# abowman6/CBET_RayTracing_3D

Hardware: AMD Instinct MI355X
Metric: ray-steps/sec, OMEGA 60-beam 256^3 sweep (higher is better)
Workload: dtype f64

## Files before the change

cbet_raytracing_3d_amd/build.py:

```python
import os
import shutil
import subprocess
import sys

PKG = os.path.dirname(os.path.abspath(__file__))
ROOT = os.path.dirname(PKG)
CSRC = os.path.join(PKG, "csrc")
LIB_DIR = os.path.join(PKG, "lib")
LIB_PATH = os.path.join(LIB_DIR, "libcbet_mi355x.so")
SOURCES = ["cbet_kernels.hip", "cbet_trace_window.hip", "cbet_trace_exit.hip", "cbet_grid_kernels.hip", "cbet_sph_modes.hip",
           "cbet_target.hip", "cbet_mesh.hip", "cbet_mesh_deposit.hip", "cbet_params.cpp", "cbet_context.cpp", "cbet_tables_abi.cpp", "cbet_trace_abi.cpp", "cbet_gain_abi.cpp",
           "cbet_host.cpp", "cbet_output.cpp", "cbet_sph_host.cpp", "cbet_target_host.cpp", "cbet_mesh_host.cpp", "cbet_mesh_deposit_host.cpp",
           "cbet_exchange_host.cpp"]
HEADERS = [os.path.join(CSRC, "cbet_device.h"), os.path.join(CSRC, "cbet_host_internal.h"), os.path.join(CSRC, "cbet_relocate.h"), os.path.join(CSRC, "cbet_trace_common.h"), os.path.join(CSRC, "cbet_trace_diag.h"), os.path.join(CSRC, "cbet_hd.h"), os.path.join(CSRC, "cbet_node_model.h"), os.path.join(CSRC, "cbet_node_kernel.h"), os.path.join(CSRC, "cbet_target_model.h"), os.path.join(CSRC, "cbet_mesh_model.h"), os.path.join(CSRC, "cbet_state_model.h"), os.path.join(CSRC, "cbet_mesh_deposit_model.h"), os.path.join(CSRC, "cbet_gain_model.h"), os.path.join(ROOT, "include", "cbet_mi355x.h"),
           os.path.join(ROOT, "include", "cbet_omega_beams.h")]

FLAGS = ["-O3", "-std=c++17", "--offload-arch=gfx950", "-ffp-contract=off", "-fPIC", "-shared",
         "-Wall", "-Wextra", "-Wno-unused-result", "-mllvm", "-structurizecfg-skip-uniform-regions=true"]


def hipcc():
    exe = shutil.which("hipcc") or "/opt/rocm/bin/hipcc"
    if not os.path.exists(exe):
        raise RuntimeError("hipcc not found (need ROCm to build the gfx950 library)")
    return exe


def is_stale():
    if not os.path.exists(LIB_PATH):
        return True
    built = os.path.getmtime(LIB_PATH)
    deps = [os.path.join(CSRC, s) for s in SOURCES] + HEADERS + [os.path.abspath(__file__),
                                                                os.path.join(ROOT, "tools", "cbet_gpu.cpp"),
                                                                os.path.join(ROOT, "tools", "cbet_reference_shaped.cpp"),
                                                                os.path.join(ROOT, "include", "cbet_reference_api.hpp")]
    return any(os.path.getmtime(d) > built for d in deps)


def build(force=False, verbose=False, extra_flags=()):
    if not force and not is_stale():
        return LIB_PATH
    os.makedirs(LIB_DIR, exist_ok=True)
    cmd = [hipcc()] + FLAGS + list(extra_flags) + [
        "-I", os.path.join(ROOT, "include"), "-I", CSRC,
        "-o", LIB_PATH] + [os.path.join(CSRC, s) for s in SOURCES] + ["-lrccl"]
    if verbose:
        print(" ".join(cmd), flush=True)
    run = subprocess.run(cmd, stderr=subprocess.PIPE, text=True)
    sys.stderr.write(run.stderr)
    if run.returncode != 0 and "structurizecfg-skip-uniform-regions" in run.stderr:
        print("build: this hipcc does not know -structurizecfg-skip-uniform-regions; building without it", flush=True)
        k = cmd.index("-structurizecfg-skip-uniform-regions=true")
        subprocess.check_call(cmd[:k - 1] + cmd[k + 1:])
    elif run.returncode != 0:
        raise subprocess.CalledProcessError(run.returncode, cmd)
    build_cli(verbose)
    build_ref_shaped(verbose)
    return LIB_PATH


CLI_PATH = os.path.join(PKG, "lib", "cbet-gpu")


def build_cli(verbose=False):
    cmd = ["g++", "-O2", "-std=c++17", "-I", os.path.join(ROOT, "include"),
           os.path.join(ROOT, "tools", "cbet_gpu.cpp"), "-o", CLI_PATH,
           "-L", LIB_DIR, "-lcbet_mi355x", "-Wl,-rpath,$ORIGIN", "-Wl,-rpath-link," + "/opt/rocm/lib"]
    if verbose:
        print(" ".join(cmd), flush=True)
    subprocess.check_call(cmd)
    return CLI_PATH


REF_SHAPED_PATH = os.path.join(PKG, "lib", "cbet-ref-shaped")


def build_ref_shaped(verbose=False):
    cmd = [hipcc(), "-O2", "-std=c++17", "-I", os.path.join(ROOT, "include"),
           os.path.join(ROOT, "tools", "cbet_reference_shaped.cpp"), "-o", REF_SHAPED_PATH,
           "-L", LIB_DIR, "-lcbet_mi355x", "-Wl,-rpath,$ORIGIN"]
    if verbose:
        print(" ".join(cmd), flush=True)
    subprocess.check_call(cmd)
    return REF_SHAPED_PATH


def build_variant(name, extra_flags=(), verbose=False):
    out_dir = os.path.join(ROOT, "build_alt")
    os.makedirs(out_dir, exist_ok=True)
    out = os.path.join(out_dir, "libcbet_%s.so" % name)
    cmd = [hipcc()] + FLAGS + list(extra_flags) + ["-I", os.path.join(ROOT, "include"), "-I", CSRC, "-o", out] + \
        [os.path.join(CSRC, s) for s in SOURCES] + ["-lrccl"]
    if verbose:
        print(" ".join(cmd), flush=True)
    subprocess.check_call(cmd)
    return out


if __name__ == "__main__":
    if len(sys.argv) > 2 and sys.argv[1] == "--variant":
        print(build_variant(sys.argv[2], sys.argv[3:], verbose=True))
    else:
        print(build(force="--force" in sys.argv, verbose=True))
```

cbet_raytracing_3d_amd/csrc/cbet_context.cpp:

```cpp
#include <algorithm>
#include <cmath>
#include <cstring>
#include <map>
#include <mutex>
#include <vector>

#include "cbet_host_internal.h"

using namespace cbet;

int cbet::check_geometry(const cbet_context *ctx, const cbet_params *p)
{
    const cbet_params &q = ctx->p;
    if (p->nx != q.nx || p->ny != q.ny || p->nz != q.nz || p->xmin != q.xmin || p->xmax != q.xmax ||
        p->ymin != q.ymin || p->ymax != q.ymax || p->zmin != q.zmin || p->zmax != q.zmax ||
        p->rays_per_zone != q.rays_per_zone || p->nbeams != q.nbeams || p->nprofile != q.nprofile ||
        p->max_threads != q.max_threads || p->threads_per_block != q.threads_per_block ||
        p->courant_mult != q.courant_mult || p->patch_order != q.patch_order || p->rim_merge != q.rim_merge)
        return fail(CBET_EINVAL, "launch parameters do not match the geometry the context was created for");
    return CBET_OK;
}

int cbet::entry_checks(const cbet_context *ctx, const cbet_params *p)
{
    if (!ctx) return fail(CBET_EINVAL, "NULL context");
    if (int rc = validate(p)) return rc;
    return check_geometry(ctx, p);
}

static std::mutex g_ctx_mu;
static std::map<int, cbet_context *> g_default_ctx;

int cbet::default_context(const cbet_params *p, cbet_context **out)
{
    int dev = 0;
    CBET_HIP(hipGetDevice(&dev));
    std::lock_guard<std::mutex> lk(g_ctx_mu);
    auto it = g_default_ctx.find(dev);
    if (it != g_default_ctx.end()) {
        if (check_geometry(it->second, p) == CBET_OK) {
            *out = it->second;
            return CBET_OK;
        }
        cbet_context_destroy(it->second);
        g_default_ctx.erase(it);
    }
    cbet_context *ctx = nullptr;
    if (int rc = cbet_context_create(&ctx, p, dev)) return rc;
    g_default_ctx[dev] = ctx;
    *out = ctx;
    return CBET_OK;
}

extern "C" {

int cbet_safeGPUAlloc(void **dst, size_t size, int gpu)
{
    if (!dst) return fail(CBET_EINVAL, "dst is NULL");
    hipError_t e = hipSetDevice(gpu);
    if (e != hipSuccess) return fail_hip(CBET_ENODEVICE, "hipSetDevice(%d): %s", gpu, hipGetErrorString(e));
    size_t free_b = 0, total_b = 0;
    e = hipMemGetInfo(&free_b, &total_b);
    if (e != hipSuccess) return fail_hip(CBET_EHIP, "Error encountered during hipMemGetInfo: %s", hipGetErrorString(e));
    if (free_b < size) return fail_hip(CBET_ENOMEM, "GPU: %d is out of memory", gpu);
    e = hipMalloc(dst, size);
    if (e != hipSuccess) return fail_hip(CBET_EHIP, "Error encountered during hipMalloc: %s", hipGetErrorString(e));
    return CBET_OK;
}

int cbet_moveToAndFromGPU(void *dst, void *src, size_t size, int gpu)
{
    if (gpu == -1) return fail_hip(CBET_ENODEVICE, "Attempting to move data that has not been assigned a GPU");
    if (size && (!dst || !src)) return fail(CBET_EINVAL, "NULL pointer");
    DeviceGuard guard;
    hipError_t e = hipSetDevice(gpu);
    if (e != hipSuccess) return fail_hip(CBET_ENODEVICE, "hipSetDevice(%d): %s", gpu, hipGetErrorString(e));
    e = hipMemcpy(dst, src, size, hipMemcpyDefault);
    if (e != hipSuccess) return fail_hip(CBET_EHIP, "Error encountered during hipMemcpy: %s", hipGetErrorString(e));
    return CBET_OK;
}

int cbet_gpuFree(void *ptr, int gpu)
{
    DeviceGuard guard;
    hipError_t e = hipSetDevice(gpu);
    if (e != hipSuccess) return fail_hip(CBET_ENODEVICE, "hipSetDevice(%d): %s", gpu, hipGetErrorString(e));
    CBET_HIP(hipFree(ptr));
    return CBET_OK;
}

int cbet_context_destroy(cbet_context *ctx)
{
    if (!ctx) return CBET_OK;
    DeviceGuard guard;
    (void)hipSetDevice(ctx->gpu);
    (void)hipFree(ctx->ne3d);
    (void)hipFree(ctx->kap3d);
    (void)hipFree(ctx->steprec);
    (void)hipFree(ctx->xlaunch);
    (void)hipFree(ctx->ylaunch);
    (void)hipFree(ctx->bounds);
    (void)hipFree(ctx->live);
    (void)hipFree(ctx->counters);
    (void)hipFree(ctx->flow_own);
    (void)hipFree(ctx->state_own);
    (void)hipFree(ctx->shift_own);
    delete ctx;
    return CBET_OK;
}

int cbet_context_set_launch_list(cbet_context *ctx, const int *list, long n)
{
    if (!ctx || !list) return fail(CBET_EINVAL, "NULL context or list");
    if (n <= 0 || n % kWave != 0) return fail(CBET_EINVAL, "a launch list is a whole number of 64-entry bundles (got %ld entries)", n);
    CBET_ENTER_DEVICE(ctx);
    CBET_HIP(hipDeviceSynchronize());
    std::vector<int> cur((size_t)ctx->nlive), want, got;
    if (ctx->nlive) CBET_HIP(hipMemcpy(cur.data(), ctx->live, cur.size() * sizeof(int), hipMemcpyDeviceToHost));
    for (int v : cur) if (v >= 0) want.push_back(v);
    for (long i = 0; i < n; ++i) {
        if (list[i] >= 0) got.push_back(list[i]);
        else if (list[i] != -1) return fail(CBET_EINVAL, "launch list entry %ld is %d (a ray id or -1)", i, list[i]);
    }
    for (long b = 0; b < n; b += kWave) {
        bool any = false;
        for (int l = 0; l < kWave; ++l) any = any || list[b + l] >= 0;
        if (!any) return fail(CBET_EINVAL, "bundle %ld of the launch list is empty", b / kWave);
    }
    std::sort(want.begin(), want.end());
    std::sort(got.begin(), got.end());
    if (want != got) return fail(CBET_EINVAL, "the launch list must hold exactly the context's live rays, each once (%zu given, %zu expected)", got.size(), want.size());
    int *fresh = nullptr;
    CBET_HIP(hipMalloc((void **)&fresh, (size_t)n * sizeof(int)));
    hipError_t e = hipMemcpy(fresh, list, (size_t)n * sizeof(int), hipMemcpyHostToDevice);
    if (e != hipSuccess) { (void)hipFree(fresh); return fail_hip(CBET_EHIP, "hipMemcpy(launch list): %s", hipGetErrorString(e)); }
    (void)hipFree(ctx->live);
    ctx->live = fresh;
    ctx->nlive = (int)n;
    return CBET_OK;
}

int cbet_context_create(cbet_context **out, const cbet_params *p, int gpu)
{
    if (!out) return fail(CBET_EINVAL, "ctx out-pointer is NULL");
    *out = nullptr;
    cbet_derived d;
    std::vector<double> xl, yl;
    std::vector<int> live;
    if (int rc = derive_launch(p, &d, xl, yl, live)) return rc;

    DeviceGuard guard;
    hipError_t e = hipSetDevice(gpu);
    if (e != hipSuccess) return fail_hip(CBET_ENODEVICE, "hipSetDevice(%d): %s", gpu, hipGetErrorString(e));
    cbet_context *ctx = new cbet_context;
    ctx->gpu = gpu;
    ctx->p = *p;
    ctx->d = d;
    ctx->nlive = (int)live.size();
    const size_t nodes = (size_t)p->nx * p->ny * p->nz;
    auto bail = [&](hipError_t err, const char *what) {
        cbet_context_destroy(ctx);
        return fail_hip(err == hipErrorOutOfMemory ? CBET_ENOMEM : CBET_EHIP, "%s: %s", what, hipGetErrorString(err));
    };
    if ((e = hipMalloc((void **)&ctx->ne3d, nodes * sizeof(double))) != hipSuccess) return bail(e, "hipMalloc(ne3d)");
    if ((e = hipMalloc((void **)&ctx->kap3d, nodes * sizeof(double))) != hipSuccess) return bail(e, "hipMalloc(kappa3d)");
    if ((e = hipMalloc((void **)&ctx->steprec, nodes * sizeof(StepRecord))) != hipSuccess) return bail(e, "hipMalloc(step records)");
    if ((e = hipMalloc((void **)&ctx->xlaunch, xl.size() * sizeof(double))) != hipSuccess) return bail(e, "hipMalloc(xlaunch)");
    if ((e = hipMalloc((void **)&ctx->ylaunch, yl.size() * sizeof(double))) != hipSuccess) return bail(e, "hipMalloc(ylaunch)");
    if ((e = hipMalloc((void **)&ctx->bounds, 6 * sizeof(double))) != hipSuccess) return bail(e, "hipMalloc(bounds)");
    {
        double hb[6];
        host_exit_planes(p, d, hb);
        if ((e = hipMemcpy(ctx->bounds, hb, sizeof hb, hipMemcpyHostToDevice)) != hipSuccess) return bail(e, "hipMemcpy(bounds)");
    }
    if ((e = hipMalloc((void **)&ctx->live, std::max<size_t>(1, live.size()) * sizeof(int))) != hipSuccess) return bail(e, "hipMalloc(live)");
    if ((e = hipMalloc((void **)&ctx->counters, kCntSlots * sizeof(unsigned long long))) != hipSuccess) return bail(e, "hipMalloc(counters)");
    if ((e = hipMemcpy(ctx->xlaunch, xl.data(), xl.size() * sizeof(double), hipMemcpyHostToDevice)) != hipSuccess) return bail(e, "hipMemcpy(xlaunch)");
    if ((e = hipMemcpy(ctx->ylaunch, yl.data(), yl.size() * sizeof(double), hipMemcpyHostToDevice)) != hipSuccess) return bail(e, "hipMemcpy(ylaunch)");
    if (!live.empty() &&
        (e = hipMemcpy(ctx->live, live.data(), live.size() * sizeof(int), hipMemcpyHostToDevice)) != hipSuccess)
        return bail(e, "hipMemcpy(live)");
    if ((e = hipMemset(ctx->counters, 0, kCntSlots * sizeof(unsigned long long))) != hipSuccess) return bail(e, "hipMemset(counters)");
    if ((e = target_upload_factors()) != hipSuccess) return bail(e, "hipMemcpyToSymbol(target factors)");
    *out = ctx;
    return CBET_OK;
}

int cbet_context_counters(cbet_context *ctx, void *stream, cbet_counters *out, int reset)
{
    if (!ctx || !out) return fail(CBET_EINVAL, "NULL context/counters");
    CBET_ENTER_DEVICE(ctx);
    hipStream_t s = (hipStream_t)stream;
    unsigned long long h[kCntSlots];
    CBET_HIP(hipMemcpyAsync(h, ctx->counters, sizeof h, hipMemcpyDeviceToHost, s));
    if (reset) CBET_HIP(hipMemsetAsync(ctx->counters, 0, sizeof h, s));
    CBET_HIP(hipStreamSynchronize(s));
    std::memset(out, 0, sizeof *out);
    out->ray_steps = h[kCntSteps];
    out->rays_traced = h[kCntRays];
    out->global_atomics = h[kCntGlobalAtomics];
    out->lds_evictions = h[kCntEvictions];
    out->wave_steps = h[kCntWaveSteps];
    out->wave_steps_miss = h[kCntWaveStepsMiss];
    out->wave_steps_wide = h[kCntWaveStepsWide];
    out->slabs_retired = h[kCntSlabsRetired];
    return CBET_OK;
}

int cbet_debug_bounds_violations(unsigned long long *out, int reset, void *stream)
{
    if (!out) return fail(CBET_EINVAL, "out is NULL");
    hipError_t e = audit_violations(out, reset != 0, (hipStream_t)stream);
    if (e == hipErrorNotSupported) return fail(CBET_EINVAL, "not a bounds-audit build (compile with -DCBET_DEBUG_BOUNDS)");
    if (e != hipSuccess) return fail_hip(CBET_EHIP, "audit_violations: %s", hipGetErrorString(e));
    return CBET_OK;
}

int cbet_context_list_length(const cbet_context *ctx, long *length)
{
    if (!ctx || !length) return fail(CBET_EINVAL, "NULL context/length");
    *length = ctx->nlive;
    return CBET_OK;
}

int cbet_context_tables(cbet_context *ctx, double **ne3d, double **kappa3d)
{
    if (!ctx) return fail(CBET_EINVAL, "NULL context");
    if (ne3d) *ne3d = ctx->ne3d;
    if (kappa3d) *kappa3d = ctx->kap3d;
    ++ctx->tables_version;
    return CBET_OK;
}

int cbet_context_step_records(const cbet_context *ctx, const void **records, unsigned long long *builds)
{
    if (!ctx) return fail(CBET_EINVAL, "NULL context");
    if (records) *records = ctx->steprec;
    if (builds) *builds = ctx->rec_builds;
    return CBET_OK;
}

int cbet_context_set_flow(cbet_context *ctx, const double *flow)
{
    if (!ctx) return fail(CBET_EINVAL, "NULL context");
    ctx->flow = flow;
    return CBET_OK;
}

int cbet_context_flow(cbet_context *ctx, void **out)
{
    if (!ctx || !out) return fail(CBET_EINVAL, "NULL context/out");
    *out = const_cast<double *>(ctx->flow);
    return CBET_OK;
}

int cbet_context_set_state(cbet_context *ctx, const double *state)
{
    if (!ctx) return fail(CBET_EINVAL, "NULL context");
    ctx->state = state;
    return CBET_OK;
}

int cbet_context_state(cbet_context *ctx, void **out)
{
    if (!ctx || !out) return fail(CBET_EINVAL, "NULL context/out");
    *out = const_cast<double *>(ctx->state);
    return CBET_OK;
}

int cbet_context_set_saturation(cbet_context *ctx, double dn_max)
{
    if (std::isnan(dn_max)) return fail(CBET_EINVAL, "cbet_context_set_saturation: dn_max is NaN (a finite limit > 0, or 0 = none)");
    if (std::isinf(dn_max)) return fail(CBET_EINVAL, "cbet_context_set_saturation: dn_max is infinite (a finite limit > 0, or 0 = none)");
    if (dn_max < 0.0) return fail(CBET_EINVAL, "cbet_context_set_saturation: dn_max = %g is negative (a finite limit > 0, or 0 = none)", dn_max);
    if (!ctx) return fail(CBET_EINVAL, "NULL context");
    ctx->dn_max = dn_max;
    return CBET_OK;
}

int cbet_context_saturation(cbet_context *ctx, double *out)
{
    if (!ctx || !out) return fail(CBET_EINVAL, "NULL context/out");
    *out = ctx->dn_max;
    return CBET_OK;
}

int cbet_context_set_detuning(cbet_context *ctx, const double *domega, int nbeams, void *stream)
{
    if (domega) {
        if (nbeams > CBET_MAX_CBET_BEAMS)
            return fail(CBET_EINVAL, "cbet_context_set_detuning: nbeams = %d exceeds CBET_MAX_CBET_BEAMS = %d", nbeams, CBET_MAX_CBET_BEAMS);
        if (nbeams < 1) return fail(CBET_EINVAL, "cbet_context_set_detuning: nbeams = %d (one shift per beam)", nbeams);
        for (int b = 0; b < nbeams; ++b) {
            if (std::isnan(domega[b])) return fail(CBET_EINVAL, "cbet_context_set_detuning: domega[%d] is NaN (finite shifts in rad/s, or NULL = none)", b);
            if (std::isinf(domega[b])) return fail(CBET_EINVAL, "cbet_context_set_detuning: domega[%d] is infinite (finite shifts in rad/s, or NULL = none)", b);
        }
    }
    if (!ctx) return fail(CBET_EINVAL, "NULL context");
    if (domega && nbeams != ctx->p.nbeams)
        return fail(CBET_EINVAL, "cbet_context_set_detuning: nbeams = %d, the context was created for %d beams", nbeams, ctx->p.nbeams);
    bool one_colour = true;
    for (int b = 1; domega && b < nbeams; ++b) one_colour = one_colour && domega[b] == domega[0];
    if (one_colour) {
        ctx->shift = nullptr;
        return CBET_OK;
    }
    CBET_ENTER_DEVICE(ctx);
    if (!ctx->shift_own) {
        hipError_t e = hipMalloc((void **)&ctx->shift_own, sizeof ctx->shift_host);
        if (e != hipSuccess) {
            ctx->shift_own = nullptr;
            return fail_hip(e == hipErrorOutOfMemory ? CBET_ENOMEM : CBET_EHIP, "hipMalloc(detuning table): %s", hipGetErrorString(e));
        }
    }
    double fresh[CBET_MAX_CBET_BEAMS] = {};
    for (int b = 0; b < nbeams; ++b) fresh[b] = domega[b];
    CBET_HIP(hipStreamSynchronize((hipStream_t)stream));
    CBET_HIP(hipMemcpy(ctx->shift_own, fresh, sizeof fresh, hipMemcpyHostToDevice));
    std::memcpy(ctx->shift_host, fresh, sizeof fresh);
    ctx->shift = ctx->shift_own;
    return CBET_OK;
}

int cbet_context_detuning(cbet_context *ctx, double *out, int *nbeams)
{
    if (!ctx || !nbeams) return fail(CBET_EINVAL, "NULL context/nbeams");
    *nbeams = ctx->shift ? ctx->p.nbeams : 0;
    if (out)
        for (int b = 0; b < *nbeams; ++b) out[b] = ctx->shift_host[b];
    return CBET_OK;
}

}
```

cbet_raytracing_3d_amd/csrc/cbet_device.h:

```cpp
#ifndef CBET_DEVICE_H_
#define CBET_DEVICE_H_

#include <hip/hip_runtime_api.h>

#include "cbet_mi355x.h"

namespace cbet {

constexpr double kC = 29979245800.0;
constexpr double kE0 = 8.85418782e-12;
constexpr double kMe = 9.10938356e-31;
constexpr double kEc = 1.60217662e-19;
constexpr double kLambda = 1.053e-4 / 3.0;
constexpr double kSigma = 0.0375;
constexpr double kIntensity = 1.0e14;
constexpr double kFocal = 0.1;
constexpr double kBeamMin = -450.0e-4;
constexpr double kBeamMax = 450.0e-4;

constexpr unsigned kEmptyTag = 0xFFFFFFFFu;
constexpr int kWave = 64;

enum CounterSlot { kCntSteps = 0, kCntRays = 1, kCntGlobalAtomics = 2, kCntEvictions = 3, kCntWaveSteps = 4,
                   kCntWaveStepsMiss = 5, kCntWaveStepsWide = 6, kCntSlabsRetired = 7, kCntSlots = 8 };

struct TabulateArgs {
    int nx, ny, nz, nprofile;
    double xmin, ymin, zmin;
    double dx, dy, dz, dt;
    double ncrit;
    const double *r, *ne, *te;
    double *ne3d, *kap3d;
};

struct StepRecord {
    double kx, ky, kz, kap;
};

struct StepTableArgs {
    int nx, ny, nz;
    double xconst, yconst, zconst;
    const double *ne3d, *kap3d;
    StepRecord *rec;
};

struct PlasmaRecordsArgs {
    TabulateArgs t;
    double xconst, yconst, zconst;
    StepRecord *rec;
};

struct TraceArgs {
    int nx, ny, nz;
    double xmin, ymin, zmin;
    double dx, dy, dz, dt;
    double inv_dx, inv_dy, inv_dz;
    double fx_hi, fy_hi, fz_hi;
    const double *bounds;
    double exit_planes[6];
    double tol_x, tol_y, tol_z;
    double xconst, yconst, zconst;
    int nt, absorption;
    int rpz, zones, nrays_x;
    double z_launch;
    double uray_mult, omega, ncrit;
    const double *xlaunch, *ylaunch;
    const int *live;
    int nlive;
    int beam_lo, nbeams_local, bundles_per_beam;
    long total_bundles;
    long first_item, item_count;
    const double *ne3d, *kap3d;
    const StepRecord *steprec;
    const double *beam_norm, *bbeam_norm, *pow_r, *phase_r;
    double *edep;
    int sYh, sXh;
    long grid_stride;
    unsigned long long *counters;
    int stats;
    unsigned long long *audit_count;
    const double *audit_lo, *audit_hi;
    unsigned long long audit_nodes, audit_hsize;
    int grid_beam0;
    const double *gain;
    long hsize;
    int quantity;
    long comp_stride;
    double max_exponent;
    double *beam_gain;
};

struct GainArgs {
    int nx, ny, nz, nbeams;
    double xmin, ymin, zmin, dx, dy, dz, dt;
    double ncrit, k0;
    double cs, gain_const, iaw;
    double mach_r0, mach_0, mach_r1, mach_1;
    double relax;
    double *fields;
    const double *ne3d;
    double *gain;
    double *scratch;
    double *change;
    int hx_lo, hx_hi;
    int consume;
    int frozen;
    long store0, bstride;
    const double *flow;
    const double *state;
    double sat;
    const double *shift;
};

hipError_t launch_tabulate(const TabulateArgs &a, hipStream_t stream);
hipError_t launch_step_table(const StepTableArgs &a, hipStream_t stream);
hipError_t launch_plasma_records(const PlasmaRecordsArgs &a, hipStream_t stream);
size_t plasma_records_lds(int nprofile);
hipError_t audit_violations(unsigned long long *out, bool reset, hipStream_t stream);
hipError_t launch_trace(const TraceArgs &a, int variant, bool force_idx64, hipStream_t stream);
hipError_t launch_trace_window(const TraceArgs &a, bool force_idx64, hipStream_t stream);
constexpr int kTraceExits = 100;
constexpr int kExitDoubles = 10;
hipError_t launch_trace_exit(const TraceArgs &a, bool force_idx64, hipStream_t stream);
hipError_t launch_exit_tally(const cbet_ray_exit *exits, long L, int nbeams, double *tally, hipStream_t stream);
hipError_t launch_farfield(const cbet_ray_exit *exits, long n, int ntheta, int nphi, double *hist, hipStream_t stream);
hipError_t launch_gain_field(const GainArgs &a, hipStream_t stream);
hipError_t launch_pair_amplitude(const GainArgs &a, double *amp, hipStream_t stream);
inline long exchange_groups(long rows) { return rows < CBET_EXCHANGE_MAX_GROUPS ? rows : CBET_EXCHANGE_MAX_GROUPS; }
hipError_t launch_exchange_matrix(const GainArgs &a, double *work, double *out, double *gross, hipStream_t stream);
hipError_t launch_pack_segments(const double *src, long beam_stride, int hy, int hz, const int *seg, long nseg, double *out,
                                hipStream_t stream);
hipError_t launch_unpack_segments(double *dst, long beam_stride, int hy, int hz, const int *seg, long nseg, const double *in,
                                  hipStream_t stream);
hipError_t launch_edep_average(const double *edep, double *out, int nx, int ny, int nz, hipStream_t stream);

struct SphArgs {
    const double *edep;
    long grid_stride;
    long row_pitch;
    int ngrids, nx, ny, nz;
    int nshell, lmax;
    double xmin, ymin, zmin, dx, dy, dz;
    double cx, cy, cz;
    double *coeffs;
    double *shell_energy;
    long long *shell_nodes;
    double r_edges[CBET_SPH_MAX_SHELLS + 1];
};
hipError_t launch_sph_modes(const SphArgs &a, hipStream_t stream);

constexpr int kTargetS = CBET_TARGET_LMAX + 1;
constexpr int kTargetCoeffs = kTargetS * kTargetS;
constexpr int kTfY00 = 0, kTfSqrt2 = 1, kTfD = 2, kTfA = kTfD + kTargetS, kTfB = kTfA + kTargetCoeffs,
              kTargetFactors = kTfB + kTargetCoeffs;
const double *target_factors();
hipError_t target_upload_factors();
struct TargetArgs {
    TabulateArgs t;
    double ox, oy, oz;
    double c[kTargetCoeffs];
};
int target_check(const cbet_target *target, int *inst);
void target_fill(const cbet_target *target, TargetArgs *a);
hipError_t launch_tabulate_target(const TargetArgs &a, int inst, hipStream_t stream);

struct FlowArgs {
    int nx, ny, nz;
    double xmin, ymin, zmin, dx, dy, dz;
    double cs, mach_r0, mach_0, mach_r1, mach_1;
    double *flow;
    double ox, oy, oz;
    double c[kTargetCoeffs];
};
hipError_t launch_tabulate_flow(const FlowArgs &a, int inst, hipStream_t stream);

struct StateConsts {
    double e2, a, f, mi_kg;
};
struct MeshArgs {
    int nx, ny, nz;
    double xmin, ymin, zmin, dx, dy, dz, dt;
    double ncrit;
    double ox, oy, oz;
    int nr, nth, nph;
    const double *r, *theta, *phi;
    const double *ne, *te;
    const double *ur, *uth, *uph;
    double *ne3d, *kap3d;
    double *flow;
    const double *ti, *zbar;
    double ti0, z0;
    StateConsts sc;
    double *state;
};
hipError_t launch_tabulate_mesh(const MeshArgs &a, hipStream_t stream);
hipError_t launch_mesh_flow(const MeshArgs &a, hipStream_t stream);
hipError_t launch_mesh_state(const MeshArgs &a, hipStream_t stream);

struct MeshDepositArgs {
    const double *edep;
    long grid_stride, row_pitch;
    int ngrids, nx, ny, nz;
    double xmin, ymin, zmin, dx, dy, dz;
    double ox, oy, oz;
    int nr, nth, nph;
    int S;
    double inv;
    const double *re, *ct, *pe, *off;
    double *cell_energy, *outside;
    long long *cell_samples;
    int chunk;
};
constexpr int kMeshDepositChunks = 8;
constexpr size_t kMeshDepositLds = 40960;
size_t mesh_deposit_lds(const MeshDepositArgs &a, bool lds_arm);
hipError_t launch_mesh_deposit(const MeshDepositArgs &a, bool lds_arm, hipStream_t stream);

}
#endif
```

cbet_raytracing_3d_amd/csrc/cbet_host_internal.h:

```cpp
#ifndef CBET_HOST_INTERNAL_H_
#define CBET_HOST_INTERNAL_H_

#include <hip/hip_runtime_api.h>

#include <vector>

#include "cbet_device.h"
#include "cbet_mi355x.h"

struct cbet_context {
    int gpu = -1;
    cbet_params p{};
    cbet_derived d{};
    double *ne3d = nullptr, *kap3d = nullptr;
    cbet::StepRecord *steprec = nullptr;
    unsigned long long tables_version = 0, rec_version = ~0ull;
    unsigned long long rec_builds = 0;
    const double *rec_ne3d = nullptr, *rec_kap3d = nullptr;
    double rec_const[3] = {0, 0, 0};
    double *xlaunch = nullptr, *ylaunch = nullptr;
    double *bounds = nullptr;
    int *live = nullptr;
    int nlive = 0;
    unsigned long long *counters = nullptr;
    double *flow_own = nullptr;
    const double *flow = nullptr;
    double *state_own = nullptr;
    const double *state = nullptr;
    double dn_max = 0.0;
    double *shift_own = nullptr;
    const double *shift = nullptr;
    double shift_host[CBET_MAX_CBET_BEAMS] = {};
};

namespace cbet {
#pragma GCC visibility push(hidden)

int fail(int code, const char *fmt, ...);
template <class... Values>
int fail_hip(int code, const char *fmt, Values... values)
{
    (void)hipGetLastError();
    return fail(code, fmt, values...);
}

#define CBET_HIP(call)                                                                          \
    do {                                                                                        \
        hipError_t e_ = (call);                                                                 \
        if (e_ != hipSuccess)                                                                   \
            return ::cbet::fail_hip(CBET_EHIP, "%s failed: %s", #call, hipGetErrorString(e_));  \
    } while (0)

struct DeviceGuard {
    int saved = -1;
    bool clear_sticky;
    explicit DeviceGuard(bool clear = false) : clear_sticky(clear) { if (hipGetDevice(&saved) != hipSuccess) saved = -1; }
    ~DeviceGuard()
    {
        if (saved >= 0) (void)hipSetDevice(saved);
        if (clear_sticky) (void)hipGetLastError();
    }
};

#define CBET_ENTER_DEVICE(context)                                                                                        \
    ::cbet::DeviceGuard device_guard_;                                                                                    \
    if (hipError_t e_ = hipSetDevice((context)->gpu))                                                                     \
        return ::cbet::fail_hip(CBET_EHIP, "hipSetDevice(ctx->gpu) failed: %s", hipGetErrorString(e_))

int validate(const cbet_params *p);
int validate_gain(const cbet_params *p, const cbet_gain_params *g);
int derive_grid(const cbet_params *p, cbet_derived *d);
int derive_launch(const cbet_params *p, cbet_derived *d, std::vector<double> &xl, std::vector<double> &yl,
                  std::vector<int> &live);
int state_consts(const cbet_params *p, const cbet_gain_params *g, StateConsts *out);

int check_geometry(const cbet_context *ctx, const cbet_params *p);
int entry_checks(const cbet_context *ctx, const cbet_params *p);
int default_context(const cbet_params *p, cbet_context **out);

template <class Args>
void grid_dims(Args &a, const cbet_params *p)
{
    a.nx = p->nx; a.ny = p->ny; a.nz = p->nz;
}
template <class Args>
void grid_args(Args &a, const cbet_params *p, const cbet_derived &d)
{
    grid_dims(a, p);
    a.xmin = p->xmin; a.ymin = p->ymin; a.zmin = p->zmin;
    a.dx = d.dx; a.dy = d.dy; a.dz = d.dz;
}
template <class Args>
void ramp_args(Args &a, const cbet_gain_params *g, double cs)
{
    a.cs = cs;
    a.mach_r0 = g->mach_r0; a.mach_0 = g->mach_0; a.mach_r1 = g->mach_r1; a.mach_1 = g->mach_1;
}
inline void host_exit_planes(const cbet_params *p, const cbet_derived &d, double out[6])
{
    out[0] = p->xmin - (d.dx / 2.0); out[1] = p->xmax + (d.dx / 2.0);
    out[2] = p->ymin - (d.dy / 2.0); out[3] = p->ymax + (d.dy / 2.0);
    out[4] = p->zmin - (d.dz / 2.0); out[5] = p->zmax + (d.dz / 2.0);
}
template <class Body>
void for_each_node_host(int nx, int ny, int nz, Body body)
{
    for (int i = 0; i < nx; ++i)
        for (int j = 0; j < ny; ++j)
            for (int k = 0; k < nz; ++k) body(i, j, k, ((long)i * ny + j) * nz + k);
}
TabulateArgs tabulate_args(const cbet_params *p, const cbet_derived &d, double *ne3d, double *kap3d, const double *te,
                           const double *r, const double *ne);
FlowArgs flow_args(const cbet_params *p, const cbet_derived &d, const cbet_gain_params *g, double cs,
                   const cbet_target *target, double *out);
MeshArgs mesh_args(const cbet_params *p, const cbet_derived &d, const cbet_mesh *mesh, double *ne3d, double *kap3d,
                   double *flow);
MeshArgs mesh_state_args(const cbet_params *p, const cbet_derived &d, const cbet_gain_params *g, const StateConsts &sc,
                         const cbet_mesh *mesh, const cbet_mesh_ions *ions, double *state);
int mesh_check(const cbet_mesh *mesh, bool whole);
GainArgs gain_args(const cbet_params *p, const cbet_derived &d, const cbet_gain_params *g, double cs, double gc,
                   const double *fields, const double *ne3d, const double *flow, const double *state, double sat,
                   const double *shift, int hx_lo, int hx_hi, bool packed);
int slab_check(const char *who, int hx_lo, int hx_hi, const cbet_params *p);

int own_node_table(double **slot, const cbet_params *p, int components, const char *what);
inline int flow_own_table(cbet_context *ctx, const cbet_params *p) { return own_node_table(&ctx->flow_own, p, 3, "flow table"); }
inline int state_own_table(cbet_context *ctx, const cbet_params *p) { return own_node_table(&ctx->state_own, p, 2, "state table"); }
int step_records(cbet_context *ctx, const cbet_params *p, const double *ne3d, const double *kappa3d, double xconst,
                 double yconst, double zconst, void *stream, bool force);
struct CbetHooks {
    const double *gain = nullptr;
    int quantity = 0;
    double *beam_gain = nullptr;
    double max_exponent = 0.0;
    bool exits = false;
};
int trace_impl(int b, unsigned nindices, const double *ne3d, const double *kappa3d, double *edep, const double *bbeam_norm,
               const double *beam_norm, const double *pow_r, const double *phase_r, double xconst, double yconst,
               double zconst, const cbet_params *p, cbet_context *ctx, void *stream, const CbetHooks &hooks);
int gain_field_impl(double *fields, const double *ne3d, double *gain, double *scratch, double *change, int hx_lo, int hx_hi,
                    bool packed, const cbet_params *p, const cbet_gain_params *g, cbet_context *ctx, void *stream,
                    bool consume = false);

#pragma GCC visibility pop
}
#endif
```

cbet_raytracing_3d_amd/csrc/cbet_kernels.hip:

```cpp
#include <hip/hip_runtime.h>

#include "cbet_node_kernel.h"
#include "cbet_node_model.h"
#include "cbet_trace_common.h"

namespace cbet {
namespace {

__device__ __forceinline__ void node_plasma(const TabulateArgs &a, const double *s_r, const double *s_ne, const double *s_te,
                                            int i, int j, int k, double &ed, double &kap)
{
    double sx, sy, sz, rho, etemp;
    node_centre(a, i, j, k, 0.0, 0.0, 0.0, sx, sy, sz, rho);
    interp2(s_ne, s_te, s_r, rho, a.nprofile, ed, etemp);
    kap = kappa(ed, etemp, a.ncrit, a.dt);
}

__global__ void __launch_bounds__(256) k_tabulate(const TabulateArgs a)
{
    extern __shared__ double s_prof[];
    double *s_r = s_prof, *s_ne = s_prof + a.nprofile, *s_te = s_prof + 2 * a.nprofile;
    for (int i = threadIdx.x; i < a.nprofile; i += blockDim.x) {
        s_r[i] = a.r[i];
        s_ne[i] = a.ne[i];
        s_te[i] = a.te[i];
    }
    __syncthreads();
    const long total = (long)a.nx * a.ny * a.nz;
    const long stride = (long)gridDim.x * blockDim.x;
    for (long idx = (long)blockIdx.x * blockDim.x + threadIdx.x; idx < total; idx += stride) {
        const int k = (int)(idx % a.nz);
        const long ij = idx / a.nz;
        const int j = (int)(ij % a.ny);
        const int i = (int)(ij / a.ny);
        double ed, kap;
        node_plasma(a, s_r, s_ne, s_te, i, j, k, ed, kap);
        a.ne3d[idx] = ed;
        a.kap3d[idx] = kap;
    }
}

__global__ void __launch_bounds__(256) k_step_table(const StepTableArgs a)
{
    const long total = (long)a.nx * a.ny * a.nz;
    const long stride = (long)gridDim.x * blockDim.x;
    const long sY = a.nz, sX = (long)a.ny * a.nz;
    for (long idx = (long)blockIdx.x * blockDim.x + threadIdx.x; idx < total; idx += stride) {
        const int k = (int)(idx % a.nz);
        const long ij = idx / a.nz;
        const int j = (int)(ij % a.ny);
        const int i = (int)(ij / a.ny);
        long oxm, oxp, oym, oyp, ozm, ozp;
        face_pair(i, a.nx, oxm, oxp, sX);
        face_pair(j, a.ny, oym, oyp, sY);
        face_pair(k, a.nz, ozm, ozp);
        StepRecord r;
        r.kx = a.xconst * (a.ne3d[idx + oxp] - a.ne3d[idx + oxm]);
        r.ky = a.yconst * (a.ne3d[idx + oyp] - a.ne3d[idx + oym]);
        r.kz = a.zconst * (a.ne3d[idx + ozp] - a.ne3d[idx + ozm]);
        r.kap = a.kap3d[idx];
        a.rec[idx] = r;
    }
}

constexpr int kPrTY = 8, kPrTZ = 64, kPrXC = 16, kPrThreads = 256;
constexpr int kPrPZ = kPrTZ + 2;
constexpr int kPrPlane = (kPrTY + 2) * kPrPZ;
constexpr int kPrTile = kPrTY * kPrTZ;
constexpr int kPrItems = kPrTile + 2 * kPrTZ + 2 * kPrTY;

__global__ void __launch_bounds__(kPrThreads) k_plasma_records(const PlasmaRecordsArgs a)
{
    extern __shared__ double s_prof[];
    const TabulateArgs &t = a.t;
    double *s_r = s_prof, *s_ne = s_prof + t.nprofile, *s_te = s_prof + 2 * t.nprofile;
    double *s_ring = s_prof + 3 * t.nprofile;
    double *s_kap = s_ring + 3 * kPrPlane;
    const int tid = threadIdx.x;
    for (int i = tid; i < t.nprofile; i += kPrThreads) {
        s_r[i] = t.r[i];
        s_ne[i] = t.ne[i];
        s_te[i] = t.te[i];
    }
    __syncthreads();
    const int nx = t.nx, ny = t.ny, nz = t.nz;
    const int k0 = max(0, min((int)blockIdx.x * kPrTZ, nz - kPrTZ));
    const int j0 = max(0, min((int)blockIdx.y * kPrTY, ny - kPrTY));
    const int x0 = (int)blockIdx.z * kPrXC, x1 = min(x0 + kPrXC, nx);
    const int pa = x0 == 0 ? 0 : min(x0 - 1, nx - 3);
    const int pb = x1 == nx ? nx : max(x1 + 1, 3);

    auto emit = [&](int i, int xl, int xh) {
        const double *lo = s_ring + (xl % 3) * kPrPlane, *hi = s_ring + (xh % 3) * kPrPlane, *mid = s_ring + (i % 3) * kPrPlane;
        const double *kap = s_kap + (i % 3) * kPrTile;
        for (int q = tid; q < 2 * kPrTile; q += kPrThreads) {
            const int n = q >> 1, jr = n / kPrTZ, kr = n % kPrTZ;
            const int j = j0 + jr, k = k0 + kr;
            if (j >= ny || k >= nz) continue;
            const int c = (jr + 1) * kPrPZ + kr + 1;
            double v0, v1;
            int m, p;
            if ((q & 1) == 0) {
                face_pair(j, ny, m, p);
                v0 = a.xconst * (hi[c] - lo[c]);
                v1 = a.yconst * (mid[c + p * kPrPZ] - mid[c + m * kPrPZ]);
            } else {
                face_pair(k, nz, m, p);
                v0 = a.zconst * (mid[c + p] - mid[c + m]);
                v1 = kap[n];
            }
            const long idx = ((long)i * ny + j) * nz + k;
            reinterpret_cast<double2 *>(a.rec + idx)[q & 1] = make_double2(v0, v1);
        }
    };

    for (int p = pa; p < pb; ++p) {
        const bool own_plane = p >= x0 && p < x1;
        double *ring = s_ring + (p % 3) * kPrPlane;
        for (int n = tid; n < (own_plane ? kPrItems : kPrTile); n += kPrThreads) {
            int jj, kk;
            if (n < kPrTile) {
                jj = 1 + n / kPrTZ; kk = 1 + n % kPrTZ;
            } else if (n < kPrTile + 2 * kPrTZ) {
                const int h = n - kPrTile;
                jj = h < kPrTZ ? 0 : kPrTY + 1; kk = 1 + h % kPrTZ;
            } else {
                const int h = n - kPrTile - 2 * kPrTZ;
                kk = h < kPrTY ? 0 : kPrTZ + 1; jj = 1 + h % kPrTY;
            }
            const int j = j0 + jj - 1, k = k0 + kk - 1;
            if (j < 0 || j >= ny || k < 0 || k >= nz) continue;
            double ed, kap;
            if (own_plane && n < kPrTile) {
                node_plasma(t, s_r, s_ne, s_te, p, j, k, ed, kap);
                s_kap[(p % 3) * kPrTile + n] = kap;
                const long idx = ((long)p * ny + j) * nz + k;
                t.ne3d[idx] = ed;
                t.kap3d[idx] = kap;
            } else {
                node_plasma(t, s_r, s_ne, s_te, p, j, k, ed, kap);
            }
            ring[jj * kPrPZ + kk] = ed;
        }
        __syncthreads();
        if (p == 2 && x0 == 0) emit(0, 0, 2);
        if (p - 1 >= 1 && p - 1 >= x0 && p - 1 < x1) emit(p - 1, p - 2, p);
        if (p == nx - 1 && x1 == nx) emit(nx - 1, nx - 3, nx - 1);
        __syncthreads();
    }
}

template <int WL>
struct LdsWindow {
    static constexpr int W = 1 << WL;
    static constexpr int NSLOT = W * W * W;
    double *val;
    unsigned *tag;
    const TraceArgs *args;

    __device__ __forceinline__ unsigned slot(int i, int j, int k) const
    {
        return (unsigned)((((i & (W - 1)) << WL) | (j & (W - 1))) << WL | (k & (W - 1)));
    }
    __device__ __forceinline__ void clear(int lane)
    {
        for (int s = lane; s < NSLOT; s += kWave) {
            val[s] = 0.0;
            tag[s] = kEmptyTag;
        }
    }
    __device__ __forceinline__ void add(unsigned s, double w)
    {
        if (CBET_AUDIT(*args, s < (unsigned)NSLOT))
            __hip_atomic_fetch_add(&val[s], w, __ATOMIC_RELAXED, __HIP_MEMORY_SCOPE_WORKGROUP);
    }
    __device__ __forceinline__ int flush(int lane, double *edep)
    {
        int n = 0;
        for (int s = lane; s < NSLOT; s += kWave) {
            const unsigned t = tag[s];
            if (t != kEmptyTag) {
                global_add(*args, &edep[t], val[s]);
                ++n;
            }
        }
        return n;
    }
};

template <int WL>
__device__ __forceinline__ void lds_deposit8(LdsWindow<WL> &win, bool pending, const unsigned (&slot)[8],
                                             const unsigned (&node)[8], const double (&w)[8],
                                             double *edep, int &n_evict)
{
    unsigned miss = 0;
    if (pending) {
        unsigned t[8];
#pragma unroll
        for (int c = 0; c < 8; ++c)
            t[c] = __hip_atomic_load(&win.tag[slot[c]], __ATOMIC_RELAXED, __HIP_MEMORY_SCOPE_WORKGROUP);
#pragma unroll
        for (int c = 0; c < 8; ++c) {
            if (t[c] == node[c])
                win.add(slot[c], w[c]);
            else
                miss |= 1u << c;
        }
    }
    if (!__any(miss != 0)) return;
    __builtin_amdgcn_wave_barrier();
#pragma unroll
    for (int c = 0; c < 8; ++c) {
        bool pend = (miss >> c) & 1u;
        while (__any(pend)) {
            unsigned t = 0;
            if (pend)
                t = __hip_atomic_load(&win.tag[slot[c]], __ATOMIC_RELAXED, __HIP_MEMORY_SCOPE_WORKGROUP);
            if (pend && t == node[c]) {
                win.add(slot[c], w[c]);
                pend = false;
            }
            __builtin_amdgcn_wave_barrier();
            if (pend) {
                unsigned expect = t;
                const bool won = __hip_atomic_compare_exchange_strong(
                    &win.tag[slot[c]], &expect, node[c], __ATOMIC_RELAXED, __ATOMIC_RELAXED,
                    __HIP_MEMORY_SCOPE_WORKGROUP);
                if (won) {
                    const unsigned long long old = __hip_atomic_exchange(
                        reinterpret_cast<unsigned long long *>(&win.val[slot[c]]),
                        (unsigned long long)__double_as_longlong(w[c]), __ATOMIC_RELAXED,
                        __HIP_MEMORY_SCOPE_WORKGROUP);
                    if (t != kEmptyTag) {
                        global_add(*win.args, &edep[t], __longlong_as_double((long long)old));
                        ++n_evict;
                    }
                    pend = false;
                }
            }
            __builtin_amdgcn_wave_barrier();
        }
    }
}

template <int DEPOSIT>
__global__ void __launch_bounds__(kWave) k_trace_simple(const TraceArgs a)
{
    constexpr int WL = 3;
    constexpr int NSLOT = DEPOSIT == 2 ? (1 << (3 * WL)) : 1;
    __shared__ double s_val[NSLOT];
    __shared__ unsigned s_tag[NSLOT];
    const int lane = threadIdx.x;
    int beam, patch;
    if (!work_item(a, blockIdx.x, beam, patch)) return;
    double *const edep = a.edep + (long)(beam - a.grid_beam0) * a.grid_stride;
    const bool absorb = a.absorption == 1;

    Ray s;
    int li;
    const bool launched = launch_lane(a, beam, patch, lane, s, li);
    bool alive = launched;

    const int nx = a.nx, ny = a.ny, nz = a.nz;
    const long sY = nz, sX = (long)ny * nz;
    const int sYh = a.sYh, sXh = a.sXh;
    int nsteps = 0, n_atomics = 0, n_evict = 0;
    unsigned wave_steps = 0;

    LdsWindow<WL> tagged{s_val, s_tag, &a};
    if (DEPOSIT == 2) {
        tagged.clear(lane);
        __syncthreads();
    }

    for (int tt = 0; tt < a.nt; ++tt) {
        if (__ballot(alive) == 0) break;
        ++wave_steps;
        unsigned slot[8] = {0, 0, 0, 0, 0, 0, 0, 0}, node[8] = {0, 0, 0, 0, 0, 0, 0, 0};
        double wgt[8] = {0, 0, 0, 0, 0, 0, 0, 0};
        if (alive) {
            int im, ip, jm, jp, km, kp;
            face_pair(s.ci, nx, im, ip);
            face_pair(s.cj, ny, jm, jp);
            face_pair(s.ck, nz, km, kp);
            auto ne_at = [&](int i, int j, int k) { return node_load<true>(a, a.ne3d, (unsigned)(i * sX + j * sY + k), a.audit_nodes); };
            s.vx -= a.xconst * (ne_at(s.ci + ip, s.cj, s.ck) - ne_at(s.ci + im, s.cj, s.ck));
            s.vy -= a.yconst * (ne_at(s.ci, s.cj + jp, s.ck) - ne_at(s.ci, s.cj + jm, s.ck));
            s.vz -= a.zconst * (ne_at(s.ci, s.cj, s.ck + kp) - ne_at(s.ci, s.cj, s.ck + km));
            double fx, fy, fz;
            drift(a, s, fx, fy, fz);
            s.ci = relocate_loop(s.ci, fx, nx);
            s.cj = relocate_loop(s.cj, fy, ny);
            s.ck = relocate_loop(s.ck, fz, nz);
            double inc;
            if (absorb) {
                inc = node_load<true>(a, a.kap3d, (unsigned)(s.ci * sX + s.cj * sY + s.ck), a.audit_nodes) * s.uray;
                s.uray -= inc;
            } else {
                inc = s.uray;
            }
            const double ox = fx - s.ci - 0.5, oy = fy - s.cj - 0.5, oz = fz - s.ck - 0.5;
            const double dm = 1.0 - fabs(ox), dn = 1.0 - fabs(oy), dl = 1.0 - fabs(oz);
            const int X0 = s.ci + 1, X1 = X0 + (ox < 0 ? -1 : 1);
            const int Y0 = s.cj + 1, Y1 = Y0 + (oy < 0 ? -1 : 1);
            const int Z0 = s.ck + 1, Z1 = Z0 + (oz < 0 ? -1 : 1);
            const double Fx0 = 1.0 - dm, Fy0 = 1.0 - dn, Fz0 = 1.0 - dl;
            const double zy00 = Fz0 * Fy0, zy10 = dl * Fy0, zy01 = Fz0 * dn, zy11 = dl * dn;
            wgt[0] = zy00 * Fx0 * inc; wgt[1] = zy00 * dm * inc; wgt[2] = zy10 * Fx0 * inc; wgt[3] = zy10 * dm * inc;
            wgt[4] = zy01 * Fx0 * inc; wgt[5] = zy01 * dm * inc; wgt[6] = zy11 * Fx0 * inc; wgt[7] = zy11 * dm * inc;
            const int nX0 = X0 * sXh, nX1 = X1 * sXh, nY0 = Y0 * sYh, nY1 = Y1 * sYh;
            node[0] = nX0 + nY0 + Z0; node[1] = nX1 + nY0 + Z0; node[2] = nX0 + nY0 + Z1; node[3] = nX1 + nY0 + Z1;
            node[4] = nX0 + nY1 + Z0; node[5] = nX1 + nY1 + Z0; node[6] = nX0 + nY1 + Z1; node[7] = nX1 + nY1 + Z1;
            if (DEPOSIT == 1) {
#pragma unroll
                for (int c = 0; c < 8; ++c) global_add(a, &edep[node[c]], wgt[c]);
                n_atomics += 8;
            } else {
                slot[0] = tagged.slot(X0, Y0, Z0); slot[1] = tagged.slot(X1, Y0, Z0);
                slot[2] = tagged.slot(X0, Y0, Z1); slot[3] = tagged.slot(X1, Y0, Z1);
                slot[4] = tagged.slot(X0, Y1, Z0); slot[5] = tagged.slot(X1, Y1, Z0);
                slot[6] = tagged.slot(X0, Y1, Z1); slot[7] = tagged.slot(X1, Y1, Z1);
            }
            ++nsteps;
        }
        if (DEPOSIT == 2) lds_deposit8<WL>(tagged, alive, slot, node, wgt, edep, n_evict);
        if (alive && stop_test(s, a.bounds) != 0) alive = false;
    }
    if (DEPOSIT == 2) {
        __syncthreads();
        n_atomics += tagged.flush(lane, edep) + n_evict;
    }
    count_steps_and_rays(a, lane, nsteps, launched);
    const int tot_at = wave_sum(n_atomics), tot_ev = wave_sum(n_evict);
    if (lane == 0) {
        atomicAdd(&a.counters[kCntGlobalAtomics], (unsigned long long)tot_at);
        atomicAdd(&a.counters[kCntEvictions], (unsigned long long)tot_ev);
        atomicAdd(&a.counters[kCntWaveSteps], (unsigned long long)wave_steps);
    }
}

#ifdef CBET_DEBUG_BOUNDS
__device__ unsigned long long g_audit_violations;
#endif

}

hipError_t launch_tabulate(const TabulateArgs &a, hipStream_t stream)
{
    const size_t lds = sizeof(double) * 3 * (size_t)a.nprofile;
    hipLaunchKernelGGL(k_tabulate, dim3(node_blocks((long)a.nx * a.ny * a.nz)), dim3(256), lds, stream, a);
    return hipGetLastError();
}

hipError_t launch_step_table(const StepTableArgs &a, hipStream_t stream)
{
    hipLaunchKernelGGL(k_step_table, dim3(node_blocks((long)a.nx * a.ny * a.nz)), dim3(256), 0, stream, a);
    return hipGetLastError();
}

size_t plasma_records_lds(int nprofile)
{
    return sizeof(double) * (3 * (size_t)nprofile + 3 * (size_t)kPrPlane + 3 * (size_t)kPrTile);
}

hipError_t launch_plasma_records(const PlasmaRecordsArgs &a, hipStream_t stream)
{
    const dim3 grid((unsigned)((a.t.nz + kPrTZ - 1) / kPrTZ), (unsigned)((a.t.ny + kPrTY - 1) / kPrTY),
                    (unsigned)((a.t.nx + kPrXC - 1) / kPrXC));
    hipLaunchKernelGGL(k_plasma_records, grid, dim3(kPrThreads), plasma_records_lds(a.t.nprofile), stream, a);
    return hipGetLastError();
}

hipError_t audit_violations(unsigned long long *out, bool reset, hipStream_t stream)
{
#ifdef CBET_DEBUG_BOUNDS
    hipError_t e = hipStreamSynchronize(stream);
    if (e != hipSuccess) return e;
    e = hipMemcpyFromSymbol(out, HIP_SYMBOL(g_audit_violations), sizeof *out);
    if (e == hipSuccess && reset) {
        const unsigned long long zero = 0;
        e = hipMemcpyToSymbol(HIP_SYMBOL(g_audit_violations), &zero, sizeof zero);
    }
    return e;
#else
    (void)out; (void)reset; (void)stream;
    return hipErrorNotSupported;
#endif
}

hipError_t launch_trace(const TraceArgs &a0, int variant, bool force_idx64, hipStream_t stream)
{
    TraceArgs a = a0;
#ifdef CBET_DEBUG_BOUNDS
    {
        const long cells = (long)(a.nx + 2) * a.sXh;
        a.audit_lo = a.edep;
        a.audit_hi = a.edep + (a.grid_stride ? a.grid_stride * (long)(a.beam_lo - a.grid_beam0 + a.nbeams_local) : cells);
        if (a.quantity != 0) a.audit_hi = a.edep + 4 * a.comp_stride;
        a.audit_nodes = (unsigned long long)a.nx * a.ny * a.nz;
        a.audit_hsize = (unsigned long long)a.hsize;
        hipError_t e = hipGetSymbolAddress((void **)&a.audit_count, HIP_SYMBOL(g_audit_violations));
        if (e != hipSuccess) return e;
    }
#endif
    if (variant == CBET_KERNEL_LDS_WINDOW) return launch_trace_window(a, force_idx64, stream);
    if (variant == kTraceExits) return launch_trace_exit(a, force_idx64, stream);
    const long waves = a.item_count;
    if (waves <= 0) return hipSuccess;
    const dim3 grid((unsigned)waves);
    if (variant == CBET_KERNEL_GLOBAL_ATOMICS) hipLaunchKernelGGL((k_trace_simple<1>), grid, dim3(kWave), 0, stream, a);
    else hipLaunchKernelGGL((k_trace_simple<2>), grid, dim3(kWave), 0, stream, a);
    return hipGetLastError();
}

}
```

cbet_raytracing_3d_amd/csrc/cbet_trace_abi.cpp:

```cpp
#include "cbet_host_internal.h"

using namespace cbet;

int cbet::trace_impl(int b, unsigned nindices, const double *ne3d, const double *kappa3d, double *edep,
                     const double *bbeam_norm, const double *beam_norm, const double *pow_r, const double *phase_r,
                     double xconst, double yconst, double zconst, const cbet_params *p, cbet_context *ctx, void *stream,
                     const CbetHooks &hooks)
{
    if (int rc = entry_checks(ctx, p)) return rc;
    if (!edep || !beam_norm || !pow_r || !phase_r) return fail(CBET_EINVAL, "NULL device pointer");
    if (nindices == 0) return CBET_OK;
    if ((int)nindices != ctx->d.nindices)
        return fail(CBET_EINVAL, "nindices=%u but def.cuh:129 gives %d for these parameters", nindices, ctx->d.nindices);

    int beam_lo = p->beam_lo, beam_hi = p->beam_hi;
    if (beam_hi >= 0 && beam_hi < beam_lo) return fail(CBET_EINVAL, "beam range [%d,%d) is reversed", beam_lo, beam_hi);
    if (beam_hi < 0) {
        const int ng = p->ngpus > 0 ? p->ngpus : 1;
        const int per = p->nbeams / ng;
        beam_lo = b * per;
        beam_hi = beam_lo + per;
    }
    if (beam_lo < 0 || beam_hi > p->nbeams || beam_hi < beam_lo)
        return fail(CBET_EINVAL, "beam range [%d,%d) outside [0,%d)", beam_lo, beam_hi, p->nbeams);
    if (beam_hi == beam_lo || ctx->nlive == 0) return CBET_OK;

    int variant = p->kernel_variant;
    if (variant == CBET_KERNEL_DEFAULT) variant = CBET_KERNEL_LDS_WINDOW;
    if (variant != CBET_KERNEL_GLOBAL_ATOMICS && variant != CBET_KERNEL_LDS_COMBINE &&
        variant != CBET_KERNEL_LDS_WINDOW)
        return fail(CBET_EINVAL, "unknown kernel_variant %d", p->kernel_variant);
    const bool cbet_hooks = hooks.gain || hooks.quantity != 0 || hooks.beam_gain;
    if (cbet_hooks && variant != CBET_KERNEL_LDS_WINDOW)
        return fail(CBET_EINVAL, "the CBET hooks exist for the default kernel (CBET_KERNEL_LDS_WINDOW) only");

    const cbet_derived &d = ctx->d;
    if (variant == CBET_KERNEL_LDS_WINDOW && d.nt >= 65536)
        return fail(CBET_EINVAL, "nt = %d steps per ray: the default kernel counts a bundle's steps in 16 bits (courant_mult too small)", d.nt);
    TraceArgs a{};
    grid_args(a, p, d);
    a.dt = d.dt;
    a.inv_dx = 1 / d.dx; a.inv_dy = 1 / d.dy; a.inv_dz = 1 / d.dz;
    a.fx_hi = p->nx - 3.0; a.fy_hi = p->ny - 3.0; a.fz_hi = p->nz - 3.0;
    a.bounds = ctx->bounds;
    host_exit_planes(&ctx->p, ctx->d, a.exit_planes);
    a.tol_x = 0.5001 * d.dx; a.tol_y = 0.5001 * d.dy; a.tol_z = 0.5001 * d.dz;
    a.xconst = xconst; a.yconst = yconst; a.zconst = zconst;
    a.nt = d.nt; a.absorption = p->absorption;
    a.rpz = p->rays_per_zone; a.zones = d.zones_spanned; a.nrays_x = d.nrays_x;
    a.z_launch = kFocal - d.dz / 2;
    a.uray_mult = d.uray_mult; a.omega = d.omega; a.ncrit = d.ncrit;
    a.xlaunch = ctx->xlaunch; a.ylaunch = ctx->ylaunch;
    a.live = ctx->live; a.nlive = ctx->nlive;
    a.beam_lo = beam_lo; a.nbeams_local = beam_hi - beam_lo;
    a.bundles_per_beam = (ctx->nlive + kWave - 1) / kWave;
    a.total_bundles = (long)a.nbeams_local * a.bundles_per_beam;
    {
        const long K = p->shard_count > 1 ? p->shard_count : 1, r = p->shard_count > 1 ? p->shard_index : 0;
        a.first_item = (r * a.total_bundles) / K;
        a.item_count = ((r + 1) * a.total_bundles) / K - a.first_item;
    }
    a.ne3d = ne3d ? ne3d : ctx->ne3d;
    a.kap3d = kappa3d ? kappa3d : ctx->kap3d;
    a.beam_norm = beam_norm; a.bbeam_norm = bbeam_norm; a.pow_r = pow_r; a.phase_r = phase_r;
    a.edep = edep;
    a.sYh = p->edep_zpitch > 0 ? p->edep_zpitch : p->nz + 2;
    a.sXh = (p->ny + 2) * a.sYh;
    if (p->edep_zpitch > 0 && (p->per_beam_grids || cbet_hooks))
        return fail(CBET_EINVAL, "edep_zpitch applies to the plain path's single deposit grid (no per-beam grids, no CBET hooks)");
    a.grid_stride = (p->per_beam_grids || hooks.quantity != 0) ? d.edep_size : 0;
    if (hooks.exits) a.grid_stride = (long)kExitDoubles * ctx->nlive;
    const int gb_n = p->grid_beams > 0 ? p->grid_beams : p->nbeams, gb_0 = p->grid_beams > 0 ? p->grid_beam0 : 0;
    if ((a.grid_stride != 0 || hooks.gain) && (beam_lo < gb_0 || beam_hi > gb_0 + gb_n))
        return fail(CBET_EINVAL, "beams [%d,%d) are not all inside the beam-resolved arrays' range [%d,%d)", beam_lo, beam_hi,
                    gb_0, gb_0 + gb_n);
    a.grid_beam0 = gb_0;
    a.comp_stride = (long)gb_n * d.edep_size;
    a.counters = ctx->counters;
    a.stats = p->window_stats != 0;
    a.gain = hooks.gain; a.hsize = d.edep_size; a.quantity = hooks.quantity;
    a.max_exponent = hooks.max_exponent; a.beam_gain = hooks.beam_gain;
    CBET_ENTER_DEVICE(ctx);
    if (variant == CBET_KERNEL_LDS_WINDOW) {
        if (int rc = step_records(ctx, p, ne3d, kappa3d, xconst, yconst, zconst, stream, false)) return rc;
        a.steprec = ctx->steprec;
    }
    CBET_HIP(launch_trace(a, hooks.exits ? kTraceExits : variant, p->force_wide_index != 0, (hipStream_t)stream));
    return CBET_OK;
}

extern "C" {

int cbet_trace_nodes(int b, unsigned nindices, const double *ne3d, const double *kappa3d,
                     double *edep, const double *bbeam_norm, const double *beam_norm,
                     const double *pow_r, const double *phase_r, double xconst, double yconst,
                     double zconst, const cbet_params *p, cbet_context *ctx, void *stream)
{
    return trace_impl(b, nindices, ne3d, kappa3d, edep, bbeam_norm, beam_norm, pow_r, phase_r, xconst, yconst,
                      zconst, p, ctx, stream, CbetHooks{});
}

int cbet_launch_ray_XYZ(int b, unsigned nindices, double *te_data_g, double *r_data_g,
                        double *ne_data_g, double *edep, double *bbeam_norm, double *beam_norm,
                        double *pow_r, double *phase_r, double xconst, double yconst,
                        double zconst, const cbet_params *p, cbet_context *ctx, void *stream)
{
    if (int rc = validate(p)) return rc;
    if (!ctx) {
        if (int rc = default_context(p, &ctx)) return rc;
    }
    const bool records = p->kernel_variant == CBET_KERNEL_DEFAULT || p->kernel_variant == CBET_KERNEL_LDS_WINDOW;
    if (int rc = records ? cbet_prepare_plasma(ctx, p, te_data_g, r_data_g, ne_data_g, xconst, yconst, zconst, stream)
                         : cbet_tabulate_plasma(ctx, p, te_data_g, r_data_g, ne_data_g, stream)) return rc;
    return cbet_trace_nodes(b, nindices, nullptr, nullptr, edep, bbeam_norm, beam_norm, pow_r, phase_r,
                            xconst, yconst, zconst, p, ctx, stream);
}

int cbet_edep_average_device(const double *edep, double *edepavg, int nx, int ny, int nz, void *stream)
{
    if (!edep || !edepavg || nx < 1 || ny < 1 || nz < 1) return fail(CBET_EINVAL, "cbet_edep_average_device: bad array");
    if ((long)(nx + 2) * (ny + 2) * (nz + 2) >= (1L << 31)) return fail(CBET_EINVAL, "cbet_edep_average_device: grid too large");
    CBET_HIP(launch_edep_average(edep, edepavg, nx, ny, nz, (hipStream_t)stream));
    return CBET_OK;
}

int cbet_trace_exits(const double *ne3d, const double *kappa3d, const double *gain, cbet_ray_exit *exits,
                     const double *bbeam_norm, const double *beam_norm, const double *pow_r, const double *phase_r,
                     double xconst, double yconst, double zconst, const cbet_params *p, const cbet_gain_params *g,
                     cbet_context *ctx, void *stream)
{
    if (int rc = validate(p)) return rc;
    if (!ctx) return fail(CBET_EINVAL, "NULL context");
    if (!exits) return fail(CBET_EINVAL, "NULL exit-record array");
    if (p->absorption != 1)
        return fail(CBET_EINVAL, "the exit pass needs absorbing mode (absorption = 1): in bookkeeping mode the increment is no energy loss");
    if (gain && !g) return fail(CBET_EINVAL, "a gain grid needs gain params (max_exponent)");
    if (g) {
        if (int rc = validate_gain(p, g)) return rc;
    }
    cbet_params q = *p;
    q.kernel_variant = CBET_KERNEL_LDS_WINDOW;
    q.per_beam_grids = 0;
    q.edep_zpitch = 0;
    q.window_stats = 0;
    if (q.beam_hi < 0) { q.beam_lo = 0; q.beam_hi = q.nbeams; }
    CbetHooks h;
    h.gain = gain; h.max_exponent = g ? g->max_exponent : 0.0; h.exits = true;
    return trace_impl(0, (unsigned)ctx->d.nindices, ne3d, kappa3d, reinterpret_cast<double *>(exits), bbeam_norm,
                      beam_norm, pow_r, phase_r, xconst, yconst, zconst, &q, ctx, stream, h);
}

int cbet_exit_tally(const cbet_ray_exit *exits, long L, int nbeams, double *tally, void *stream)
{
    if (!exits || !tally) return fail(CBET_EINVAL, "NULL exit records / tally");
    if (L < 0 || nbeams < 0) return fail(CBET_EINVAL, "L = %ld, nbeams = %d", L, nbeams);
    CBET_HIP(launch_exit_tally(exits, L, nbeams, tally, (hipStream_t)stream));
    return CBET_OK;
}

int cbet_farfield(const cbet_ray_exit *exits, long n, int ntheta, int nphi, double *hist, void *stream)
{
    if (!exits || !hist) return fail(CBET_EINVAL, "NULL exit records / histogram");
    if (n < 0 || ntheta <= 0 || nphi <= 0) return fail(CBET_EINVAL, "n = %ld, ntheta = %d, nphi = %d", n, ntheta, nphi);
    CBET_HIP(launch_farfield(exits, n, ntheta, nphi, hist, (hipStream_t)stream));
    return CBET_OK;
}

}
```

cbet_raytracing_3d_amd/csrc/cbet_trace_common.h:

```cpp
#ifndef CBET_TRACE_COMMON_H_
#define CBET_TRACE_COMMON_H_

#include <hip/hip_runtime.h>

#include "cbet_device.h"
#include "cbet_relocate.h"

namespace cbet {

__device__ __forceinline__ double interp_table(const double *y, const double *x, const double xp, int n)
{
    unsigned lo, hi, mid;
    if (x[0] <= x[n - 1]) {
        if (xp <= x[0]) return y[0];
        if (xp >= x[n - 1]) return y[n - 1];
        lo = 0;
        hi = n - 1;
        mid = (lo + hi) >> 1;
        while (lo < hi - 1) {
            if (x[mid] >= xp) hi = mid; else lo = mid;
            mid = (lo + hi) >> 1;
        }
    } else {
        if (xp >= x[0]) return y[0];
        if (xp <= x[n - 1]) return y[n - 1];
        lo = 0;
        hi = n - 1;
        mid = (lo + hi) >> 1;
        while (lo < hi - 1) {
            if (x[mid] <= xp) lo = mid; else hi = mid;
            mid = (lo + hi) >> 1;
        }
    }
    return y[mid] + (y[mid + 1] - y[mid]) / (x[mid + 1] - x[mid]) * (xp - x[mid]);
}

struct Ray {
    double px, py, pz, vx, vy, vz, uray, ustop;
    int ci, cj, ck;
};

__device__ __forceinline__ int first_node_within(double p, double lo, double d, double tol, int n)
{
    double f = (p - lo) / d;
    int g = (f > -4.0 && f < (double)n + 4.0) ? (int)floor(f) : -8;
    int found = 0;
    bool have = false;
    for (int q = g - 2; q <= g + 2; ++q) {
        if (q < 0 || q >= n || have) continue;
        if (fabs(q * d + lo - p) <= tol) {
            found = q;
            have = true;
        }
    }
    return found;
}

__device__ __forceinline__ bool launch_ray(const TraceArgs &a, int beam, int pre_raynum, Ray &s)
{
    const int rpz = a.rpz, rpz2 = rpz * rpz;
    const int tile = pre_raynum / rpz2, within = pre_raynum % rpz2;
    const int ry = tile / a.zones * rpz + within / rpz;
    const int rx = tile % a.zones * rpz + within % rpz;
    double x0 = a.xlaunch[rx];
    double y0 = a.ylaunch[ry];
    const double ref = sqrt(x0 * x0 + y0 * y0);
    double z0 = a.z_launch;

    const double bnx = a.beam_norm[beam * 3 + 0], bny = a.beam_norm[beam * 3 + 1],
                 bnz = a.beam_norm[beam * 3 + 2];
    double c1, s1, c2, s2;
    if (a.bbeam_norm) {
        c1 = a.bbeam_norm[4 * beam + 0];
        s1 = a.bbeam_norm[4 * beam + 1];
        c2 = a.bbeam_norm[4 * beam + 2];
        s2 = a.bbeam_norm[4 * beam + 3];
    } else {
        const double theta1 = acos(bnz);
        const double theta2 = atan2(bny * kFocal, kFocal * bnx);
        c1 = cos(theta1);
        s1 = sin(theta1);
        c2 = cos(theta2);
        s2 = sin(theta2);
    }
    const double keep = x0;
    x0 = x0 * c1 + z0 * s1;
    z0 = z0 * c1 - keep * s1;
    const double keep2 = x0;
    x0 = x0 * c2 - y0 * s2;
    y0 = y0 * c2 + keep2 * s2;

    s.px = x0;
    s.py = y0;
    s.pz = z0;
    s.uray = a.uray_mult * interp_table(a.pow_r, a.phase_r, ref, CBET_NPHASE);
    s.ustop = 0.05 * s.uray;
    if (!(ref <= kBeamMax)) return false;

    s.ci = first_node_within(s.px, a.xmin, a.dx, a.tol_x, a.nx);
    s.cj = first_node_within(s.py, a.ymin, a.dy, a.tol_y, a.ny);
    s.ck = first_node_within(s.pz, a.zmin, a.dz, a.tol_z, a.nz);

    const double ne0 = a.ne3d[((long)s.ci * a.ny + s.cj) * a.nz + s.ck];
    const double w = sqrt((a.omega * a.omega - ne0 * 1e6 * (kEc * kEc) / ((double)kMe * kE0)) / (kC * kC));
    double vx = -1 * bnx, vy = -1 * bny, vz = -1 * bnz;
    const double knorm = sqrt(vx * vx + vy * vy + vz * vz);
    s.vx = (kC * kC) * ((vx / knorm) * w) / a.omega;
    s.vy = (kC * kC) * ((vy / knorm) * w) / a.omega;
    s.vz = (kC * kC) * ((vz / knorm) * w) / a.omega;
    return true;
}

__device__ __forceinline__ bool launch_lane(const TraceArgs &a, int beam, int patch, int lane, Ray &s, int &li)
{
    li = patch * kWave + lane;
    const int pre_raynum = li < a.nlive ? a.live[li] : -1;
    return pre_raynum >= 0 && launch_ray(a, beam, pre_raynum, s);
}

template <class T = int> __device__ __forceinline__ void face_pair(int c, int n, T &m, T &p, T stride = 1)
{
    m = (c == 0) ? 0 : ((c == n - 1) ? -2 * stride : -stride);
    p = (c == 0) ? 2 * stride : ((c == n - 1) ? 0 : stride);
}

__device__ __forceinline__ void drift(const TraceArgs &a, Ray &s, double &fx, double &fy, double &fz)
{
    s.px += s.vx * a.dt; s.py += s.vy * a.dt; s.pz += s.vz * a.dt;
    fx = (s.px - a.xmin) * a.inv_dx; fy = (s.py - a.ymin) * a.inv_dy; fz = (s.pz - a.zmin) * a.inv_dz;
}

__device__ __forceinline__ int stop_test(const Ray &s, const double *b)
{
    const bool out = s.px < b[0] || s.px > b[1] || s.py < b[2] || s.py > b[3] || s.pz < b[4] || s.pz > b[5];
    return (s.uray <= s.ustop ? CBET_RAY_CUTOFF : 0) | (out ? CBET_RAY_ESCAPED : 0);
}

#ifdef CBET_DEBUG_BOUNDS
__device__ __forceinline__ bool audit_fail(const TraceArgs &a)
{
    atomicAdd(a.audit_count, 1ull);
    return true;
}
#define CBET_AUDIT(a, cond) ((cond) || !audit_fail(a))
#else
#define CBET_AUDIT(a, cond) true
#endif

__device__ __forceinline__ void global_add(const TraceArgs &a, double *p, double v)
{
#ifdef CBET_DEBUG_BOUNDS
    if (!(p >= a.audit_lo && p < a.audit_hi)) { audit_fail(a); return; }
#else
    (void)a;
#endif
    unsafeAtomicAdd(p, v);
}

__device__ __forceinline__ int wave_sum(int v)
{
#pragma unroll
    for (int off = 32; off > 0; off >>= 1) v += __shfl_xor(v, off, 64);
    return v;
}
__device__ __forceinline__ void count_steps_and_rays(const TraceArgs &a, int lane, int steps, bool launched)
{
    const int tot_steps = wave_sum(launched ? steps : 0), tot_rays = wave_sum(launched ? 1 : 0);
    if (lane == 0) {
        atomicAdd(&a.counters[kCntSteps], (unsigned long long)tot_steps);
        atomicAdd(&a.counters[kCntRays], (unsigned long long)tot_rays);
    }
}

template <bool IDX64>
__device__ __forceinline__ double node_load(const TraceArgs &a, const double *base, unsigned idx, unsigned long long bound)
{
#ifdef CBET_DEBUG_BOUNDS
    if (!(idx < bound)) { audit_fail(a); return 0.0; }
#else
    (void)a; (void)bound;
#endif
    if (IDX64) return base[idx];
    return *reinterpret_cast<const double *>(reinterpret_cast<const char *>(base) + (idx * 8u));
}

typedef double gain_pair_t __attribute__((ext_vector_type(2), aligned(8)));
template <bool IDX64>
__device__ __forceinline__ gain_pair_t gain_load2(const TraceArgs &a, const double *base, unsigned idx)
{
#ifdef CBET_DEBUG_BOUNDS
    if (!(idx + 1u < a.audit_hsize)) { audit_fail(a); return gain_pair_t{0.0, 0.0}; }
#else
    (void)a;
#endif
    if (IDX64) return *reinterpret_cast<const gain_pair_t *>(base + idx);
    return *reinterpret_cast<const gain_pair_t *>(reinterpret_cast<const char *>(base) + (idx * 8u));
}

__device__ __forceinline__ double phi_det(double x)
{
    double p = 1.0 / 6402373705728000.0;
    p = p * x + 1.0 / 355687428096000.0;
    p = p * x + 1.0 / 20922789888000.0;
    p = p * x + 1.0 / 1307674368000.0;
    p = p * x + 1.0 / 87178291200.0;
    p = p * x + 1.0 / 6227020800.0;
    p = p * x + 1.0 / 479001600.0;
    p = p * x + 1.0 / 39916800.0;
    p = p * x + 1.0 / 3628800.0;
    p = p * x + 1.0 / 362880.0;
    p = p * x + 1.0 / 40320.0;
    p = p * x + 1.0 / 5040.0;
    p = p * x + 1.0 / 720.0;
    p = p * x + 1.0 / 120.0;
    p = p * x + 1.0 / 24.0;
    p = p * x + 1.0 / 6.0;
    p = p * x + 0.5;
    p = p * x + 1.0;
    return p;
}

__device__ __forceinline__ double phi_small(double x)
{
    double p = 1.0 / 40320.0;
    p = __builtin_fma(p, x, 1.0 / 5040.0);
    p = __builtin_fma(p, x, 1.0 / 720.0);
    p = __builtin_fma(p, x, 1.0 / 120.0);
    p = __builtin_fma(p, x, 1.0 / 24.0);
    p = __builtin_fma(p, x, 1.0 / 6.0);
    p = __builtin_fma(p, x, 0.5);
    p = __builtin_fma(p, x, 1.0);
    return p;
}

__device__ __forceinline__ double sqrt_speed(double v2)
{
    const double r0 = __builtin_amdgcn_rsq(v2);
    double g = v2 * r0, h = 0.5 * r0;
    const double e = __builtin_fma(-h, g, 0.5);
    g = __builtin_fma(g, e, g); h = __builtin_fma(h, e, h);
    g = __builtin_fma(__builtin_fma(-g, g, v2), h, g);
    return __builtin_fma(__builtin_fma(-g, g, v2), h, g);
}

__device__ __forceinline__ void factor_pair(double o, int flip, double &f0, double &f1)
{
    const double g = fabs(o) - (double)flip;
    f0 = __hiloint2double(__double2hiint(g) ^ (flip << 31), __double2loint(g));
    f1 = 1.0 - f0;
}

template <bool IDX64>
__device__ __forceinline__ double gain_exponent(const TraceArgs &a, const double *gk, int X0, int X1, int Y0, int Y1, int Z0, int Z1, double Fx0,
                                                double Fx1, double Fy0, double Fy1, double Fz0, double Fz1, int sXh, int sYh, double ds)
{
    const int nX0 = __mul24(X0, sXh), nX1 = __mul24(X1, sXh), nY0 = __mul24(Y0, sYh), nY1 = __mul24(Y1, sYh);
    const bool z0_low = Z0 < Z1;
    const int zl = z0_low ? Z0 : Z1;
    const double fz_lo = z0_low ? Fz0 : Fz1, fz_hi = z0_low ? Fz1 : Fz0;
    const gain_pair_t c00 = gain_load2<IDX64>(a, gk, (unsigned)(nX0 + nY0 + zl)), c10 = gain_load2<IDX64>(a, gk, (unsigned)(nX1 + nY0 + zl));
    const gain_pair_t c01 = gain_load2<IDX64>(a, gk, (unsigned)(nX0 + nY1 + zl)), c11 = gain_load2<IDX64>(a, gk, (unsigned)(nX1 + nY1 + zl));
    const double q00 = __builtin_fma(fz_hi, c00.y, fz_lo * c00.x), q10 = __builtin_fma(fz_hi, c10.y, fz_lo * c10.x);
    const double q01 = __builtin_fma(fz_hi, c01.y, fz_lo * c01.x), q11 = __builtin_fma(fz_hi, c11.y, fz_lo * c11.x);
    const double r0 = __builtin_fma(Fx1, q10, Fx0 * q00), r1 = __builtin_fma(Fx1, q11, Fx0 * q01);
    const double ksum = __builtin_fma(Fy1, r1, Fy0 * r0);
    double x = ksum * ds;
    if (x > a.max_exponent) x = a.max_exponent;
    if (x < -a.max_exponent) x = -a.max_exponent;
    return x;
}

constexpr double kPhiSmallBelow = 0.03125;
__device__ __forceinline__ double gain_phi(double x, bool wave_is_small) { return wave_is_small ? phi_small(x) : phi_det(x); }

__device__ __forceinline__ bool work_item(const TraceArgs &a, long w, int &beam, int &patch)
{
    const long g = a.first_item + w;
    if (w >= a.item_count) return false;
    const int beam_local = (int)(g / a.bundles_per_beam);
    patch = (int)(g - (long)beam_local * a.bundles_per_beam);
    beam = a.beam_lo + beam_local;
    return true;
}

}
#endif
```

cbet_raytracing_3d_amd/csrc/cbet_trace_diag.h:

```cpp
#ifndef CBET_TRACE_DIAG_H_
#define CBET_TRACE_DIAG_H_

#include "cbet_trace_common.h"

namespace cbet {

#ifdef CBET_DIAG_CLOCKS
#define CBET_IF_CLOCKS(...) __VA_ARGS__
#else
#define CBET_IF_CLOCKS(...)
#endif
#ifdef CBET_DIAG_FACES
#define CBET_IF_FACES(...) __VA_ARGS__
#else
#define CBET_IF_FACES(...)
#endif
#ifdef CBET_DIAG_CHAIN
#define CBET_IF_CHAIN(...) __VA_ARGS__
#else
#define CBET_IF_CHAIN(...)
#endif

struct WaveDiag {
    typedef unsigned long long u64;
    static constexpr bool kCountsWaveSteps = (0 CBET_IF_CLOCKS(+1) CBET_IF_FACES(+1) CBET_IF_CHAIN(+1)) != 0;
    CBET_IF_CLOCKS(u64 wait = 0, arm = 0, n_arm = 0, ret = 0, n_ret = 0, t_start, t_wait, t_arm, t_ret;)
    CBET_IF_FACES(unsigned near_steps = 0, near_axes = 0, arm_steps = 0;)
    CBET_IF_CHAIN(u64 chain = 0, t_chain = 0;)

    static __device__ __forceinline__ void stamp(u64 &t) { asm volatile("s_memtime %0" : "=&s"(t) : : "memory"); }
    static __device__ __forceinline__ void stamp_wait(u64 &t) { asm volatile("s_memtime %0\n\ts_waitcnt lgkmcnt(0)" : "=&s"(t) : : "memory"); }
    static __device__ __forceinline__ u64 since(u64 t0)
    {
        u64 t1;
        asm volatile("s_memtime %0\n\ts_waitcnt lgkmcnt(0)" : "=&s"(t1) : "s"(t0) : "memory");
        return t1 - t0;
    }

    __device__ __forceinline__ void begin() { CBET_IF_CLOCKS(stamp_wait(t_start);) }
    __device__ __forceinline__ void step_begin(int near)
    {
        (void)near;
        CBET_IF_FACES(near_steps += near != 0 ? 1 : 0; near_axes += __builtin_popcount((unsigned)near);)
    }
    __device__ __forceinline__ void wait_begin() { CBET_IF_CLOCKS(stamp(t_wait);) }
    __device__ __forceinline__ void wait_end()
    {
        CBET_IF_CLOCKS(wait += since(t_wait);)
        CBET_IF_CHAIN(stamp_wait(t_chain);)
    }
    __device__ __forceinline__ void chain_end() { CBET_IF_CHAIN(chain += since(t_chain);) }
    __device__ __forceinline__ void arm_begin()
    {
        CBET_IF_FACES(arm_steps += 1;)
        CBET_IF_CLOCKS(stamp(t_arm);)
    }
    __device__ __forceinline__ void arm_end() { CBET_IF_CLOCKS(arm += since(t_arm); n_arm += 1;) }
    __device__ __forceinline__ void retire_begin() { CBET_IF_CLOCKS(stamp(t_ret);) }
    __device__ __forceinline__ void retire_end() { CBET_IF_CLOCKS(ret += since(t_ret); n_ret += 1;) }
    __device__ __forceinline__ bool report(const TraceArgs &a, int lane, int tot_steps, int tot_rays, unsigned wave_steps)
    {
        auto put = [&](int slot, u64 v) { atomicAdd(&a.counters[slot], v); };
        if (kCountsWaveSteps && lane == 0) {
            CBET_IF_CLOCKS(u64 t_end; stamp_wait(t_end);)
            put(kCntSteps, (u64)tot_steps);
            put(kCntWaveSteps, (u64)wave_steps);
#if defined(CBET_DIAG_CLOCKS)
            put(kCntGlobalAtomics, wait);
            put(kCntEvictions, arm);
            put(kCntWaveStepsWide, n_arm);
            put(kCntSlabsRetired, t_end - t_start);
            put(kCntRays, ret);
            put(kCntWaveStepsMiss, n_ret);
#elif defined(CBET_DIAG_CHAIN)
            put(kCntRays, (u64)tot_rays);
            put(kCntGlobalAtomics, chain);
#elif defined(CBET_DIAG_FACES)
            put(kCntRays, (u64)tot_rays);
            put(kCntWaveStepsWide, (u64)near_steps);
            put(kCntWaveStepsMiss, (u64)near_axes);
            put(kCntSlabsRetired, (u64)arm_steps);
#endif
        }
        (void)tot_rays;
        return kCountsWaveSteps;
    }
};
#undef CBET_IF_CLOCKS
#undef CBET_IF_FACES
#undef CBET_IF_CHAIN

}

#endif
```

cbet_raytracing_3d_amd/csrc/cbet_trace_window.hip:

```cpp
#include <hip/hip_runtime.h>

#include <cstddef>
#include <type_traits>

#if defined(__HIP_DEVICE_COMPILE__) && !defined(__gfx950__)
#error "cbet_trace_window.hip is written for gfx950 (CDNA4) only"
#endif

#include "cbet_trace_common.h"
#include "cbet_trace_diag.h"

namespace cbet {
namespace {

#define CBET_BALLOT(cond) __builtin_amdgcn_ballot_w64(cond)
#define CBET_LANES(mask) __builtin_amdgcn_inverse_ballot_w64(mask)
#define CBET_USUAL(cond) __builtin_expect(!!(cond), 1)
#define CBET_RARE(cond) __builtin_expect(!!(cond), 0)
#define CBET_SELDOM(cond) __builtin_expect_with_probability(!!(cond), 0, 0.9)

template <int WX_, int WY_, int WZ_, bool PAD, bool XORSW = false>
struct Tile {
    static constexpr int WX = WX_, WY = WY_, WZ = WZ_;
    static constexpr int XM = WX - 1, YM = WY - 1, ZM = WZ - 1;
    static constexpr bool ROT = PAD && WZ == 16;
    static constexpr int YS = (PAD && !ROT) ? WZ + 1 : WZ;
    static constexpr int XS = (PAD && !ROT) ? WY * YS + 4 : WY * WZ;
    static constexpr bool XOR = ROT && XORSW;
    static __device__ __forceinline__ int zr(int tx, int ty, int tz)
    {
        return XOR ? (tz ^ ((tx & 3) << 2) ^ (ty << 1)) : (ROT ? ((tz + 7 * tx + 3 * ty) & ZM) : tz);
    }
    static_assert(!XOR || (WX == 8 && WY == 8 && WZ == 16), "the swizzle terms are written for the 8 x 8 x 16 box");
    static __device__ __forceinline__ int xterm(int tx) { return __mul24(tx, XS * 8 + 32) & ~0x80; }
    static __device__ __forceinline__ int yterm(int ty) { return __mul24(ty, YS * 8 + 16); }
    static constexpr int N = WX * XS;
    static constexpr int SX = WX - 2, SY = WY - 2, SZ = WZ - 2;
    static constexpr bool BRICK = WZ == 16 && WY == 8;
    static constexpr int DT = WX * WY * WZ;
    static __device__ __forceinline__ int slot_d(int tx, int ty, int tz) { return (tx * WY + ty) * WZ + tz; }
};

struct Origin {
    int x, y, z;
};

template <int M>
__device__ __forceinline__ int abs_in(int o, int r) { return o + ((r - o) & M); }

template <int C>
struct Corner {
    static constexpr int index = C;
    template <class V> static __device__ __forceinline__ V x(V v0, V v1) { return (C & 1) ? v1 : v0; }
    template <class V> static __device__ __forceinline__ V z(V v0, V v1) { return (C & 2) ? v1 : v0; }
    template <class V> static __device__ __forceinline__ V y(V v0, V v1) { return (C & 4) ? v1 : v0; }
};
template <class F>
__device__ __forceinline__ void each_corner(F f)
{
    f(Corner<0>{}); f(Corner<1>{}); f(Corner<2>{}); f(Corner<3>{}); f(Corner<4>{}); f(Corner<5>{}); f(Corner<6>{}); f(Corner<7>{});
}

struct WaveCounters {
    int n_atomics = 0;
    int n_miss = 0;
    unsigned steps_miss = 0;
    unsigned slabs_bsteps = 0;
    int pend = 0;
    [[no_unique_address]] WaveDiag dg;
};

template <bool W32>
struct Grid {
    double *p;
};
template <bool W32>
__device__ __forceinline__ void grid_add(const TraceArgs &a, Grid<W32> g, int node, double v)
{
    if constexpr (W32) global_add(a, reinterpret_cast<double *>(reinterpret_cast<char *>(g.p) + ((unsigned)node * 8u)), v);
    else global_add(a, &g.p[node], v);
}
template <bool W32>
__device__ __forceinline__ void grid_add_far(const TraceArgs &a, Grid<W32> g, long index, double v) { global_add(a, &g.p[index], v); }

template <class G>
__device__ __forceinline__ void write_back(const TraceArgs &a, double *tile, int slot, G edep, int node, double v, WaveCounters &wc)
{
    wc.pend += (CBET_BALLOT(v != 0.0) != 0ull) ? 1 : 0;
    if (v != 0.0) {
        tile[slot] = 0.0;
        ++wc.n_atomics;
        grid_add(a, edep, node, v);
    }
}
template <class G>
__device__ __forceinline__ void write_back_far(const TraceArgs &a, double *tile, int slot, G edep, long index, double v, WaveCounters &wc)
{
    wc.pend += (CBET_BALLOT(v != 0.0) != 0ull) ? 1 : 0;
    if (v != 0.0) {
        grid_add_far(a, edep, index, v);
        tile[slot] = 0.0;
        ++wc.n_atomics;
    }
}

template <class F>
__device__ __forceinline__ void miss_add8(unsigned long long hbm_m, WaveCounters &wc, F add8)
{
    if (CBET_RARE(hbm_m != 0ull)) {
        wc.pend += 8;
        if (CBET_LANES(hbm_m)) add8();
    }
}

template <class T, int AX, int COUNT, class G>
__device__ __forceinline__ void retire_planes(const TraceArgs &a, double *tile, const Origin &o, int coord, int step,
                                              int lane, G edep, int sXh, int sYh, WaveCounters &wc)
{
    constexpr int WO = AX == 0 ? T::WY : T::WX, OM = WO - 1;
    constexpr int IT = (WO * T::WZ + kWave - 1) / kWave;
    constexpr int RS = kWave / T::WZ;
    static_assert(IT == 1 || (IT == 2 && 2 * RS == WO), "a plane is one entry per lane, or two in the halves of the other axis");
    static_assert(!T::XOR || IT == 1 || (RS == 4 && T::YS == 16 && T::XS == 128), "the second entry's slot is written for the 8 x 8 x 16 box");
    constexpr int SLOT_X = AX == 0 ? (RS * T::YS) ^ ((2 * RS) & T::ZM) : RS * T::XS;
    const int r0 = lane / T::WZ, r1 = lane & T::ZM, k = abs_in<T::ZM>(o.z, r1);
    const int d0 = (r0 - (AX == 0 ? o.y : o.x)) & OM, dnode = ((d0 & RS) ? -RS : RS) * (AX == 0 ? sYh : sXh);
    const bool in_plane = !(WO * T::WZ < kWave) || lane < WO * T::WZ;
    double v[COUNT * IT];
    int slot[COUNT * IT], node[COUNT * IT];
#pragma unroll
    for (int pl = 0; pl < COUNT; ++pl) {
        const int c = coord + pl * step;
        const int fixed = c & (AX == 0 ? T::XM : T::YM);
#pragma unroll
        for (int e = 0; e < IT; ++e) {
            const int q = pl * IT + e, re = r0 + e * RS;
            if (e == 1 && T::XOR) {
                slot[q] = slot[q - 1] ^ SLOT_X;
                node[q] = node[q - 1] + dnode;
            } else if (AX == 0) {
                slot[q] = fixed * T::XS + re * T::YS + T::zr(fixed, re, r1);
                node[q] = c * sXh + __mul24(abs_in<T::YM>(o.y, re), sYh) + k;
            } else {
                slot[q] = re * T::XS + fixed * T::YS + T::zr(re, fixed, r1);
                node[q] = __mul24(abs_in<T::XM>(o.x, re), sXh) + c * sYh + k;
            }
            const bool ok = in_plane && CBET_AUDIT(a, (unsigned)slot[q] < (unsigned)T::N);
            v[q] = ok ? tile[slot[q]] : 0.0;
        }
    }
#pragma unroll
    for (int q = 0; q < COUNT * IT; ++q) write_back(a, tile, slot[q], edep, node[q], v[q], wc);
}

template <class T, int AX, int NC, class G>
__device__ __forceinline__ void retire_plane(const TraceArgs &a, double *tile, const Origin &o, int coord, int lane,
                                             G edep, int sXh, int sYh, WaveCounters &wc, int coff, long gstride)
{
    constexpr int WO = AX == 0 ? T::WY : T::WX;
    constexpr int IT = (WO * T::WZ + kWave - 1) / kWave;
    const int fixed = coord & (AX == 0 ? T::XM : T::YM);
#pragma unroll
    for (int e = 0; e < IT; ++e) {
        const int idx = e * kWave + lane;
        const bool in_plane = !(WO * T::WZ < kWave) || idx < WO * T::WZ;
        const int r0 = idx / T::WZ, r1 = idx & T::ZM;
        int slot, node, slot_d;
        const int k = abs_in<T::ZM>(o.z, r1);
        if (AX == 0) {
            slot = fixed * T::XS + r0 * T::YS + T::zr(fixed, r0, r1);
            slot_d = T::slot_d(fixed, r0, r1);
            node = coord * sXh + __mul24(abs_in<T::YM>(o.y, r0), sYh) + k;
        } else {
            slot = r0 * T::XS + fixed * T::YS + T::zr(r0, fixed, r1);
            slot_d = T::slot_d(r0, fixed, r1);
            node = __mul24(abs_in<T::XM>(o.x, r0), sXh) + coord * sYh + k;
        }
        const bool ok = in_plane && CBET_AUDIT(a, (unsigned)slot < (unsigned)T::N);
        const double v = ok ? tile[slot] : 0.0;
        if (NC > 1) {
#pragma unroll
            for (int q = 1; q < NC; ++q) {
                const int sq = coff + (q - 1) * T::DT + slot_d;
                write_back_far(a, tile, sq, edep, q * gstride + node, ok ? tile[sq] : 0.0, wc);
            }
        }
        write_back(a, tile, slot, edep, node, v, wc);
    }
}

template <class T, int NC, class G>
__device__ __forceinline__ void retire_zplane(const TraceArgs &a, double *tile, const Origin &o, int coord, int lane,
                                              G edep, int sXh, int sYh, WaveCounters &wc, int coff, long gstride)
{
    static_assert(T::WX * T::WY <= kWave, "one z-plane entry per lane");
    const int r0 = lane / T::WY, r1 = lane & T::YM, fixed = coord & T::ZM;
    const int slot = r0 * T::XS + r1 * T::YS + T::zr(r0, r1, fixed);
    const int node = __mul24(abs_in<T::XM>(o.x, r0), sXh) + __mul24(abs_in<T::YM>(o.y, r1), sYh) + coord;
    const bool ok = (!(T::WX * T::WY < kWave) || lane < T::WX * T::WY) && CBET_AUDIT(a, (unsigned)slot < (unsigned)T::N);
    const double v = ok ? tile[slot] : 0.0;
    if (NC > 1) {
        const int slot_d = T::slot_d(r0, r1, fixed);
#pragma unroll
        for (int q = 1; q < NC; ++q) {
            const int sq = coff + (q - 1) * T::DT + slot_d;
            write_back_far(a, tile, sq, edep, q * gstride + node, ok ? tile[sq] : 0.0, wc);
        }
    }
    write_back(a, tile, slot, edep, node, v, wc);
}

template <class T, class G>
__device__ __forceinline__ void retire_zbrick(const TraceArgs &a, double *tile, const Origin &o, int zb, int lane,
                                              G edep, int sXh, int sYh, WaveCounters &wc)
{
    static_assert(T::WY == 8 && T::WZ == 16, "a brick is 8 rows of 8 planes per tile x index");
    const int ty = lane >> 3, kz = lane & 7;
    const int tz = (zb + kz) & T::ZM;
    const int base_node = __mul24(abs_in<T::YM>(o.y, ty), sYh) + zb + kz;
    constexpr int ROUND = 4;
#pragma unroll
    for (int t0 = 0; t0 < T::WX; t0 += ROUND) {
        double v[ROUND];
        int slot[ROUND];
#pragma unroll
        for (int q = 0; q < ROUND; ++q) {
            slot[q] = (t0 + q) * T::XS + ty * T::YS + T::zr(t0 + q, ty, tz);
            v[q] = CBET_AUDIT(a, (unsigned)slot[q] < (unsigned)T::N) ? tile[slot[q]] : 0.0;
        }
#pragma unroll
        for (int q = 0; q < ROUND; ++q) write_back(a, tile, slot[q], edep, abs_in<T::XM>(o.x, t0 + q) * sXh + base_node, v[q], wc);
    }
}

template <class T, int NC, class G>
__device__ __forceinline__ void flush_box(const TraceArgs &a, double *tile, const Origin &o, int lane, G edep,
                                          int sXh, int sYh, WaveCounters &wc, int coff, long gstride)
{
    for (int t = 0; t < T::WX; ++t)
        retire_plane<T, 0, NC>(a, tile, o, o.x + t, lane, edep, sXh, sYh, wc, coff, gstride);
}

__device__ __forceinline__ int follow_plane_axis(int r, unsigned long long mm, int S)
{
    const unsigned long long edge = __builtin_amdgcn_ballot_w64((unsigned)(r - 1) >= (unsigned)(S - 1)) & mm;
    if (CBET_USUAL(edge == 0ull)) return 0;
    const unsigned long long hi = __builtin_amdgcn_ballot_w64(r >= S) & edge;
    const bool at_hi = hi != 0ull, at_lo = hi != edge;
    if (at_hi == at_lo) return 0;
    if (at_hi) {
        if ((__builtin_amdgcn_ballot_w64(r <= 1) & mm) != 0ull) return (__builtin_amdgcn_ballot_w64(r > S) & mm) != 0ull ? 1 : 0;
        return (S >= 6 && (__builtin_amdgcn_ballot_w64(r <= 2) & mm) == 0ull) ? 2 : 1;
    }
    if ((__builtin_amdgcn_ballot_w64(r >= S - 1) & mm) != 0ull) return (__builtin_amdgcn_ballot_w64(r < 0) & mm) != 0ull ? -1 : 0;
    return (S >= 6 && (__builtin_amdgcn_ballot_w64(r >= S - 2) & mm) == 0ull) ? -2 : -1;
}

__device__ __forceinline__ int follow_brick_axis(int r, unsigned long long mm)
{
    if ((__builtin_amdgcn_ballot_w64((unsigned)r > 14u) & mm) == 0ull) return 0;
    const bool below = (__builtin_amdgcn_ballot_w64(r < 0) & mm) != 0ull, above = (__builtin_amdgcn_ballot_w64(r > 14) & mm) != 0ull;
    const bool needs_lo = (__builtin_amdgcn_ballot_w64(r <= 7) & mm) != 0ull, needs_hi = (__builtin_amdgcn_ballot_w64(r >= 7) & mm) != 0ull;
    return (below && !needs_hi) ? -1 : ((above && !needs_lo) ? 1 : 0);
}

template <class T, int NC, class G>
__device__ __forceinline__ bool follow_box(const TraceArgs &a, double *tile, Origin &o, unsigned long long mm, int lx,
                                           int ly, int lz, int lane, G edep, int sXh, int sYh, WaveCounters &wc,
                                           int coff, long gstride)
{
    auto leave = [&](auto axis, int d, int lo, int hi) {
        constexpr int AX = decltype(axis)::value;
        const int first = d < 0 ? hi : lo, step = d < 0 ? -1 : 1, n = d < 0 ? -d : d;
        if constexpr (NC == 1) {
            if (n == 2) retire_planes<T, AX, 2>(a, tile, o, first, step, lane, edep, sXh, sYh, wc);
            else retire_planes<T, AX, 1>(a, tile, o, first, step, lane, edep, sXh, sYh, wc);
        } else {
            for (int q = 0; q < n; ++q) retire_plane<T, AX, NC>(a, tile, o, first + q * step, lane, edep, sXh, sYh, wc, coff, gstride);
        }
    };
    const int dx = follow_plane_axis(lx - o.x, mm, T::SX);
    const int dy = follow_plane_axis(ly - o.y, mm, T::SY);
    if (dx != 0) { wc.dg.retire_begin(); leave(std::integral_constant<int, 0>{}, dx, o.x, o.x + T::WX - 1); wc.dg.retire_end(); }
    o.x += dx;
    if (dy != 0) { wc.dg.retire_begin(); leave(std::integral_constant<int, 1>{}, dy, o.y, o.y + T::WY - 1); wc.dg.retire_end(); }
    o.y += dy;
    int dz;
    if constexpr (T::BRICK) {
        dz = 8 * follow_brick_axis(lz - o.z, mm);
        if (dz != 0) { wc.dg.retire_begin(); retire_zbrick<T>(a, tile, o, dz < 0 ? o.z + 8 : o.z, lane, edep, sXh, sYh, wc); wc.dg.retire_end(); }
    } else {
        dz = follow_plane_axis(lz - o.z, mm, T::SZ);
        if (dz != 0)
            retire_zplane<T, NC>(a, tile, o, dz < 0 ? o.z + T::WZ - 1 : o.z, lane, edep, sXh, sYh, wc, coff, gstride);
        for (int q = 1; q < (dz < 0 ? -dz : dz); ++q)
            retire_zplane<T, NC>(a, tile, o, dz < 0 ? o.z + T::WZ - 1 - q : o.z + q, lane, edep, sXh, sYh, wc, coff, gstride);
    }
    o.z += dz;
    const bool moved = (dx | dy | dz) != 0;
    wc.slabs_bsteps += moved ? (1u << 16) : 0u;
    return moved;
}

template <class T>
__device__ __forceinline__ bool holds(const Origin &o, int lx, int ly, int lz)
{
    return (unsigned)(lx - o.x) <= (unsigned)T::SX && (unsigned)(ly - o.y) <= (unsigned)T::SY &&
           (unsigned)(lz - o.z) <= (unsigned)T::SZ;
}

template <class T>
__device__ __forceinline__ int box_near_axes(const Origin &o, int nx, int ny, int nz)
{
    const int lo = kRelocateDeep + 1;
    const unsigned tx = (unsigned)((o.x - lo) | (nx - 3 - T::SX - o.x)), ty = (unsigned)((o.y - lo) | (ny - 3 - T::SY - o.y)),
                   tz = (unsigned)((o.z - lo) | (nz - 3 - T::SZ - o.z));
    return (int)((tx >> 31) | ((ty >> 31) << 1) | ((tz >> 31) << 2));
}

typedef double dbl2 __attribute__((ext_vector_type(2)));

template <bool WIDE>
__device__ __forceinline__ void record_issue(const StepRecord *base, unsigned cell, dbl2 &kxy, dbl2 &kzk)
{
    if constexpr (WIDE) {
        const char *p = reinterpret_cast<const char *>(base) + ((unsigned long long)cell << 5);
        asm volatile("global_load_dwordx4 %0, %2, off\n\tglobal_load_dwordx4 %1, %2, off offset:16\n\t; CBET_RECORD_ISSUE %0 %1"
                     : "=&v"(kxy), "=&v"(kzk)
                     : "v"(p)
                     : "memory");
    } else {
        const unsigned off = cell << 5;
        asm volatile("s_nop 4\n\tglobal_load_dwordx4 %0, %2, %3\n\tglobal_load_dwordx4 %1, %2, %3 offset:16\n\t; CBET_RECORD_ISSUE %0 %1"
                     : "=&v"(kxy), "=&v"(kzk)
                     : "v"(off), "s"(base)
                     : "memory");
    }
}

__device__ __forceinline__ void record_wait(dbl2 &kxy, dbl2 &kzk, int pend)
{
    asm volatile("; CBET_RECORD_WAIT %0 %1\n\t"
                 "s_cmp_eq_u32 %2, 0\n\t"
                 "s_cbranch_scc1 .Lrw_0_%=\n\t"
                 "s_cmp_ge_u32 %2, 8\n\t"
                 "s_cbranch_scc1 .Lrw_8_%=\n\t"
                 "s_cmp_ge_u32 %2, 4\n\t"
                 "s_cbranch_scc1 .Lrw_4_%=\n\t"
                 "s_cmp_ge_u32 %2, 2\n\t"
                 "s_cbranch_scc1 .Lrw_2_%=\n\t"
                 "s_waitcnt vmcnt(1)\n\t"
                 "s_branch .Lrw_end_%=\n"
                 ".Lrw_2_%=:\n\t"
                 "s_waitcnt vmcnt(2)\n\t"
                 "s_branch .Lrw_end_%=\n"
                 ".Lrw_4_%=:\n\t"
                 "s_waitcnt vmcnt(4)\n\t"
                 "s_branch .Lrw_end_%=\n"
                 ".Lrw_8_%=:\n\t"
                 "s_waitcnt vmcnt(8)\n\t"
                 "s_branch .Lrw_end_%=\n"
                 ".Lrw_0_%=:\n\t"
                 "s_waitcnt vmcnt(0)\n"
                 ".Lrw_end_%=:"
                 : "+v"(kxy), "+v"(kzk)
                 : "s"(pend)
                 : "memory", "scc");
}

__device__ __forceinline__ void record_wait_all(dbl2 &kxy, dbl2 &kzk)
{
    asm volatile("; CBET_RECORD_WAIT %0 %1\n\ts_waitcnt vmcnt(0)" : "+v"(kxy), "+v"(kzk) : : "memory");
}

__device__ __forceinline__ void exit_planes_load(dbl2 &bx, dbl2 &by, dbl2 &bz)
{
    const void *args = (const void *)__builtin_amdgcn_kernarg_segment_ptr();
    asm volatile("s_load_dwordx4 %0, %3, %4\n\ts_load_dwordx4 %1, %3, %5\n\ts_load_dwordx4 %2, %3, %6\n\ts_waitcnt lgkmcnt(0)"
                 : "=&s"(bx), "=&s"(by), "=&s"(bz)
                 : "s"(args), "i"(offsetof(TraceArgs, exit_planes)), "i"(offsetof(TraceArgs, exit_planes) + 16),
                   "i"(offsetof(TraceArgs, exit_planes) + 32));
}

__device__ __forceinline__ int add3(int a, int b, int c)
{
    int r;
    asm("v_add3_u32 %0, %1, %2, %3" : "=v"(r) : "v"(a), "v"(b), "v"(c));
    return r;
}

__device__ __forceinline__ int xad1(int f, int c)
{
    int r;
    asm("v_xad_u32 %0, %1, 1, %2" : "=v"(r) : "v"(f), "v"(c));
    return r;
}

__device__ __forceinline__ double max_abs3(double a, double b, double c)
{
    double r;
    asm("v_max_f64 %0, |%1|, |%2|" : "=v"(r) : "v"(a), "v"(b));
    asm("v_max_f64 %0, %1, |%2|" : "=v"(r) : "v"(r), "v"(c));
    return r;
}

__device__ __forceinline__ void commit(int &var, int value)
{
    asm volatile("s_mov_b32 %0, %1" : "+s"(var) : "s"(__builtin_amdgcn_readfirstlane(value)));
}
__device__ __forceinline__ void commit(unsigned long long &var, unsigned long long value)
{
    asm volatile("s_mov_b64 %0, %1" : "+s"(var) : "s"(value));
}
__device__ __forceinline__ void commit_v(int &var, int value) { asm volatile("v_mov_b32 %0, %1" : "+v"(var) : "v"(value)); }

__device__ __forceinline__ void cell_step(int &c, unsigned long long up, unsigned long long dn)
{
    asm("s_nop 1\n\tv_addc_co_u32_e64 %0, vcc, 0, %0, %1\n\tv_subbrev_co_u32_e64 %0, vcc, 0, %0, %2" : "+v"(c) : "s"(up), "s"(dn) : "vcc");
}
__device__ __forceinline__ void cell_step3(int &ci, int &cj, int &ck, unsigned long long upx, unsigned long long dnx,
                                           unsigned long long upy, unsigned long long dny, unsigned long long upz,
                                           unsigned long long dnz)
{
    asm("s_nop 1\n\t"
        "v_addc_co_u32_e64 %0, vcc, 0, %0, %3\n\tv_addc_co_u32_e64 %1, vcc, 0, %1, %5\n\tv_addc_co_u32_e64 %2, vcc, 0, %2, %7\n\t"
        "v_subbrev_co_u32_e64 %0, vcc, 0, %0, %4\n\tv_subbrev_co_u32_e64 %1, vcc, 0, %1, %6\n\tv_subbrev_co_u32_e64 %2, vcc, 0, %2, %8"
        : "+v"(ci), "+v"(cj), "+v"(ck)
        : "s"(upx), "s"(dnx), "s"(upy), "s"(dny), "s"(upz), "s"(dnz)
        : "vcc");
}

__device__ __forceinline__ int mad24(int a, int b, int c)
{
    int r;
    asm("s_nop 1\n\tv_mad_i32_i24 %0, %1, %2, %3" : "=v"(r) : "v"(a), "s"(b), "v"(c));
    return r;
}


#ifdef CBET_DEBUG_BOUNDS
constexpr bool kAudited = true;
#else
constexpr bool kAudited = false;
#endif
constexpr double kNearTol = 0.5001;
constexpr double kFarJump = 1.4998;

template <int WZ, bool GENERIC, int CBET, bool STATS>
__global__ void __launch_bounds__(kWave, (CBET == 4) ? 1 : 4) k_trace_window(const TraceArgs a)
{
    using T = Tile<8, 8, WZ, true, CBET == 0>;
    using TB = Tile<4, 8, 8, false>;
    constexpr bool IDX64 = GENERIC;
    constexpr int NC = (CBET == 4) ? 4 : 1;
    constexpr bool ACC = (CBET == 0);
    constexpr bool PIPE = ACC;
    constexpr int NSLOT = T::N + TB::N;
    constexpr int NLDS = NSLOT + (NC - 1) * T::DT;
    __shared__ double s_val[NLDS];
    const int lane = threadIdx.x;

    int beam, patch;
    if (!work_item(a, blockIdx.x, beam, patch)) return;
    const Grid<!IDX64> edep{a.edep + (long)(beam - a.grid_beam0) * a.grid_stride};
    const bool absorb = GENERIC ? (a.absorption == 1) : true;

    Ray s = {};
    int li;
    const bool launched = launch_lane(a, beam, patch, lane, s, li);
    unsigned long long live = __ballot(launched);
    if (live == 0ull) return;
    const int tot_rays = __popcll(live);

    const int nx = a.nx, ny = a.ny, nz = a.nz;
    const int sYh = a.sYh, sXh = a.sXh;
    unsigned cell = launched ? (unsigned)((s.ci * ny + s.cj) * nz + s.ck) : 0u;
    double fcx = (double)s.ci, fcy = (double)s.cj, fcz = (double)s.ck;
    int tot_steps = 0;
    WaveCounters wc;

    double *const tileA = s_val, *const tileB = s_val + T::N;
    Origin oA{0, 0, 0}, oB{0, 0, 0};
    unsigned long long hbm = 0ull;
    int b_active = 0;
    {
        const int src = ((live >> 27) & 1ull) ? 27 : (__ffsll((long long)live) - 1);
        for (int z = lane; z < NLDS; z += kWave) s_val[z] = 0.0;
        oA.x = __builtin_amdgcn_readlane(s.ci, src) + 1 - T::WX / 2;
        oA.y = __builtin_amdgcn_readlane(s.cj, src) + 1 - T::WY / 2;
        oA.z = __builtin_amdgcn_readlane(s.ck, src) + 1 - 4;
        if (T::BRICK) oA.z &= ~7;
        __syncthreads();
    }
    int near = 7;
    wc.dg.begin();

    dbl2 rec_kxy, rec_kzk;
    const StepRecord *rec_base = a.steprec;
    asm volatile("" : "+s"(rec_base));
    double dt = a.dt;
    auto gather_record = [&]() {
        unsigned c = CBET_LANES(live) ? cell : 0u;
        asm("" : "+v"(c));
#ifdef CBET_DEBUG_BOUNDS
        if (!(c < a.audit_nodes)) { audit_fail(a); c = 0u; }
#endif
        record_issue<IDX64>(rec_base, c, rec_kxy, rec_kzk);
        wc.pend = 0;
    };
    auto await_record = [&]() {
        wc.dg.wait_begin();
        if (CBET == 0 && !kAudited) record_wait(rec_kxy, rec_kzk, wc.pend);
        else record_wait_all(rec_kxy, rec_kzk);
        wc.dg.wait_end();
    };
    gather_record();
    await_record();
    const double *const gk = CBET && a.gain ? a.gain + (long)(beam - a.grid_beam0) * a.hsize : nullptr;
    double gained = 0.0;

    const bool flx = (lane & 1) != 0, fly = (lane & 2) != 0, flz = (lane & 8) != 0;
    const int pfx = flx ? 1 : 0, pfy = fly ? 1 : 0, pfz = flz ? 1 : 0;

    double q0 = 0.0, q1 = 0.0, q2 = 0.0, q3 = 0.0;

    int slow = 7;
    double Fx0 = 0, Fx1 = 0, Fy0 = 0, Fy1 = 0, Fz0 = 0, Fz1 = 0;
    int X0 = 0, X1 = 0, Y0 = 0, Y1 = 0, Z0 = 0, Z1 = 0;
    double inc = 0.0;
    int tile_off = 0;
    unsigned long long miss_m = 0ull;
    int own_slot = 0, own_node = 0;
    auto lds_add8 = [&](const double *w) {
        auto add = [&](int byte, double v) {
            if (CBET_AUDIT(a, (unsigned)byte < (unsigned)NSLOT * 8u))
                __hip_atomic_fetch_add(static_cast<double *>(__builtin_assume_aligned(reinterpret_cast<char *>(s_val) + byte, 8)),
                                       v, __ATOMIC_RELAXED, __HIP_MEMORY_SCOPE_WORKGROUP);
        };
        if constexpr (T::XOR) {
            int ax0, ax1, by0, by1, cz0, cz1;
            if (CBET_USUAL(b_active == 0)) {
                ax0 = T::xterm(X0 & T::XM); ax1 = T::xterm(X1 & T::XM);
                by0 = T::yterm(Y0 & T::YM); by1 = T::yterm(Y1 & T::YM);
                cz0 = (Z0 & T::ZM) << 3; cz1 = (Z1 & T::ZM) << 3;
            } else {
                const bool toB = tile_off != 0;
                const int xm = toB ? TB::XM : T::XM, zm = toB ? TB::ZM : T::ZM;
                const int xmul = toB ? TB::XS * 8 : T::XS * 8 + 32, ymul = toB ? TB::YS * 8 : T::YS * 8 + 16;
                const int keep = toB ? ~0 : ~0x80, off8 = tile_off * 8;
                static_assert(TB::YM == T::YM, "one y mask for both boxes");
                ax0 = (__mul24(X0 & xm, xmul) & keep) | off8; ax1 = (__mul24(X1 & xm, xmul) & keep) | off8;
                by0 = __mul24(Y0 & T::YM, ymul); by1 = __mul24(Y1 & T::YM, ymul);
                cz0 = (Z0 & zm) << 3; cz1 = (Z1 & zm) << 3;
            }
            auto at = [](int ax, int by, int cz) { return (int)__builtin_amdgcn_bitop3_b32(ax, by, cz, 0x96); };
            each_corner([=](auto c) { add(at(c.x(ax0, ax1), c.y(by0, by1), c.z(cz0, cz1)), w[c.index]); });
        } else {
            auto add8 = [&](int xm, int ym, int zm, int xs, int ys, int off, int rot) {
                const int xa = X0 & xm, xb = X1 & xm, ya = Y0 & ym, yb = Y1 & ym;
                const int x0 = __mul24(xa, xs * 8) + off * 8, x1 = __mul24(xb, xs * 8) + off * 8;
                const int y0 = __mul24(ya, ys * 8), y1 = __mul24(yb, ys * 8);
                const int ra = 7 * xa * rot, rb = 7 * xb * rot, sa = 3 * ya * rot, sb = 3 * yb * rot;
                auto zb = [&](int z, int r) { return ((z + r) & zm) * 8; };
                if constexpr (T::ROT) {
                    const int xy00 = x0 | y0, xy10 = x1 | y0, xy01 = x0 | y1, xy11 = x1 | y1, zm8 = zm * 8;
                    auto at = [&](int xy, int z, int r) { return (((z + r) * 8) & zm8) | xy; };
                    each_corner([&](auto c) {
                        add(at(c.y(c.x(xy00, xy10), c.x(xy01, xy11)), c.z(Z0, Z1), c.x(ra, rb) + c.y(sa, sb)), w[c.index]);
                    });
                } else {
                    each_corner([&](auto c) {
                        add(add3(c.x(x0, x1), c.y(y0, y1), zb(c.z(Z0, Z1), c.x(ra, rb) + c.y(sa, sb))), w[c.index]);
                    });
                }
            };
            if (b_active == 0) {
                add8(T::XM, T::YM, T::ZM, T::XS, T::YS, 0, T::ROT ? 1 : 0);
            } else {
                const bool toB = tile_off != 0;
                add8(toB ? TB::XM : T::XM, toB ? TB::YM : T::YM, toB ? TB::ZM : T::ZM, toB ? TB::XS : T::XS,
                     toB ? TB::YS : T::YS, tile_off, (T::ROT && !toB) ? 1 : 0);
            }
        }
    };
    auto hbm_add8 = [&](const double *w) {
        const int nX0 = __mul24(X0, sXh), nX1 = __mul24(X1, sXh), nY0 = __mul24(Y0, sYh), nY1 = __mul24(Y1, sYh);
        each_corner([&](auto c) { grid_add(a, edep, c.x(nX0, nX1) + c.y(nY0, nY1) + c.z(Z0, Z1), w[c.index]); });
        wc.n_atomics += 8;
    };

    auto deposit_step = [&](unsigned long long lds_m, unsigned long long hbm_m) {
        const double zi0 = Fz0 * inc, zi1 = Fz1 * inc;
        const double zy00 = zi0 * Fy0, zy10 = zi1 * Fy0, zy01 = zi0 * Fy1, zy11 = zi1 * Fy1;
        double wgt[8];
        wgt[0] = zy00 * Fx0;
        wgt[1] = zy00 * Fx1;
        wgt[2] = zy10 * Fx0;
        wgt[3] = zy10 * Fx1;
        wgt[4] = zy01 * Fx0;
        wgt[5] = zy01 * Fx1;
        wgt[6] = zy11 * Fx0;
        wgt[7] = zy11 * Fx1;
        if (CBET_LANES(lds_m)) lds_add8(wgt);
        miss_add8(hbm_m, wc, [&]() {
            hbm_add8(wgt);
            ++wc.n_miss;
        });
        if (CBET == 4) {
            const bool inbox = CBET_LANES(lds_m);
            if (inbox && tile_off == 0) {
                if (CBET_AUDIT(a, (unsigned)(own_slot + 2 * T::DT) < (unsigned)NLDS)) {
                    __hip_atomic_fetch_add(&s_val[own_slot], q1, __ATOMIC_RELAXED, __HIP_MEMORY_SCOPE_WORKGROUP);
                    __hip_atomic_fetch_add(&s_val[own_slot + T::DT], q2, __ATOMIC_RELAXED, __HIP_MEMORY_SCOPE_WORKGROUP);
                    __hip_atomic_fetch_add(&s_val[own_slot + 2 * T::DT], q3, __ATOMIC_RELAXED, __HIP_MEMORY_SCOPE_WORKGROUP);
                }
            } else if (inbox || CBET_LANES(hbm_m)) {
                grid_add_far(a, edep, a.comp_stride + own_node, q1);
                grid_add_far(a, edep, 2 * a.comp_stride + own_node, q2);
                grid_add_far(a, edep, 3 * a.comp_stride + own_node, q3);
                wc.n_atomics += 3;
            }
        }
    };

    double S[8] = {0, 0, 0, 0, 0, 0, 0, 0};
    unsigned long long restart_m = 0ull;
    bool p_odd = true;
    auto accumulate = [&]() {
        const double zi0 = Fz0 * inc, zi1 = Fz1 * inc;
        const double zy00 = zi0 * Fy0, zy10 = zi1 * Fy0, zy01 = zi0 * Fy1, zy11 = zi1 * Fy1;
        const double k = CBET_LANES(restart_m) ? 0.0 : 1.0;
        auto add = [&](double &sum, double w) { asm("v_fma_f64 %0, %0, %1, %2" : "+v"(sum) : "v"(k), "v"(w)); };
        add(S[0], zy00 * Fx0);
        add(S[1], zy00 * Fx1);
        add(S[2], zy10 * Fx0);
        add(S[3], zy10 * Fx1);
        add(S[4], zy01 * Fx0);
        add(S[5], zy01 * Fx1);
        add(S[6], zy11 * Fx0);
        add(S[7], zy11 * Fx1);
    };
    auto flush_sums = [&](unsigned long long lds_m, unsigned long long hbm_m) {
        if (CBET_LANES(lds_m)) lds_add8(S);
        miss_add8(hbm_m, wc, [&]() { hbm_add8(S); });
    };

    auto step_tail = [&](int &tt) {
    asm volatile("" : "+v"(Fx0), "+v"(Fx1), "+v"(Fy0), "+v"(Fy1), "+v"(Fz0), "+v"(Fz1));
    await_record();
    if (absorb) {
        inc = rec_kzk.y * s.uray;
        s.uray -= inc;
    } else {
        inc = s.uray;
    }
    if (CBET >= 2) inc = q0;
    if constexpr (ACC && !PIPE) accumulate();
    unsigned long long died = CBET_BALLOT(s.uray <= s.ustop);
    const int faces = slow | near;
    if (CBET_RARE(faces != 0)) {
        dbl2 bx, by, bz;
        exit_planes_load(bx, by, bz);
        if (faces & 1) died |= CBET_BALLOT(s.px < bx.x) | CBET_BALLOT(s.px > bx.y);
        if (faces & 2) died |= CBET_BALLOT(s.py < by.x) | CBET_BALLOT(s.py > by.y);
        if (faces & 4) died |= CBET_BALLOT(s.pz < bz.x) | CBET_BALLOT(s.pz > bz.y);
    }
    died &= live;
    if (CBET_SELDOM(died != 0ull)) {
        asm volatile("");
        commit(tot_steps, tot_steps + __popcll(died) * (tt + 1));
        if constexpr (PIPE) {
            accumulate();
            asm volatile("v_mov_b64 %0, 0" : "+v"(inc));
            commit(restart_m, 0ull);
        }
        if constexpr (ACC) flush_sums(died & ~miss_m, died & miss_m);
        else deposit_step(died & ~miss_m, died & miss_m);
        commit(live, live & ~died);
        commit(hbm, hbm & live);
        commit(miss_m, miss_m & live);
        if (live == 0ull) commit(tt, a.nt - 1);
    }
    __builtin_amdgcn_wave_barrier();
    };

    for (int tt = 0; tt < a.nt; ++tt) {
        if constexpr (STATS || WaveDiag::kCountsWaveSteps) wc.steps_miss += 1u << 16;
        wc.dg.step_begin(near);
        s.vx -= rec_kxy.x;
        s.vy -= rec_kxy.y;
        s.vz -= rec_kzk.x;
        asm volatile("" : "+s"(dt));
        s.px += s.vx * dt;
        s.py += s.vy * dt;
        s.pz += s.vz * dt;
        const double fx = (s.px - a.xmin) * a.inv_dx;
        const double fy = (s.py - a.ymin) * a.inv_dy;
        const double fz = (s.pz - a.zmin) * a.inv_dz;
        const double g0x = fx - fcx, g0y = fy - fcy, g0z = fz - fcz;
        const unsigned long long upx = CBET_BALLOT(g0x >= kNearTol), dnx = CBET_BALLOT(g0x < kNearTol - 1.0),
                                 upy = CBET_BALLOT(g0y >= kNearTol), dny = CBET_BALLOT(g0y < kNearTol - 1.0),
                                 upz = CBET_BALLOT(g0z >= kNearTol), dnz = CBET_BALLOT(g0z < kNearTol - 1.0);
        slow = ((CBET_BALLOT(!(max_abs3(g0x, g0y, g0z) < kFarJump)) & live) != 0ull) ? 7 : near;
        if (CBET_USUAL(slow == 0)) {
            cell_step3(s.ci, s.cj, s.ck, upx, dnx, upy, dny, upz, dnz);
        } else {
            if (slow & 1) s.ci = relocate_closed(s.ci, fx, nx);
            else cell_step(s.ci, upx, dnx);
            if (slow & 2) s.cj = relocate_closed(s.cj, fy, ny);
            else cell_step(s.cj, upy, dny);
            if (slow & 4) s.ck = relocate_closed(s.ck, fz, nz);
            else cell_step(s.ck, upz, dnz);
        }
        const unsigned new_cell = (unsigned)mad24(mad24(s.ci, ny, s.cj), nz, s.ck);
        unsigned long long moved_m = 0ull;
        if constexpr (ACC) moved_m = CBET_BALLOT(new_cell != cell);
        cell = new_cell;
        gather_record();
        wc.dg.chain_end();
        asm volatile("" : "+v"(s.ci), "+v"(s.cj), "+v"(s.ck), "+v"(inc));
        fcx = (double)s.ci;
        fcy = (double)s.cj;
        fcz = (double)s.ck;
        if constexpr (!ACC) deposit_step(live & ~miss_m, miss_m);
        if constexpr (PIPE) accumulate();
        const double ox = (fx - fcx) - 0.5, oy = (fy - fcy) - 0.5, oz = (fz - fcz) - 0.5;
        const bool ngx = ox < 0, ngy = oy < 0, ngz = oz < 0;
        const bool all_negative = (live & ~(CBET_BALLOT(ngx) & CBET_BALLOT(ngy) & CBET_BALLOT(ngz))) == 0ull;
        if constexpr (ACC) {
            const unsigned long long fl_m = (all_negative && !p_odd) ? (live & moved_m) : live;
            if (CBET_USUAL(fl_m != 0ull)) {
                if (CBET_USUAL(miss_m == 0ull)) flush_sums(fl_m, 0ull);
                else flush_sums(fl_m & ~miss_m, fl_m & miss_m);
            }
            restart_m = fl_m;
            p_odd = !all_negative;
        }
        factor_pair(ox, pfx, Fx0, Fx1);
        factor_pair(oy, pfy, Fy0, Fy1);
        factor_pair(oz, pfz, Fz0, Fz1);
        int rx, ry, rz;
        if (CBET_USUAL(all_negative)) {
            rx = s.ci - oA.x;
            ry = s.cj - oA.y;
            rz = s.ck - oA.z;
            asm("" : "+v"(rx), "+v"(ry), "+v"(rz));
            X0 = xad1(pfx, s.ci); X1 = s.ci + pfx;
            Y0 = xad1(pfy, s.cj); Y1 = s.cj + pfy;
            Z0 = xad1(pfz, s.ck); Z1 = s.ck + pfz;
        } else {
            const int lx = s.ci + 1 - (ngx ? 1 : 0);
            const int ly = s.cj + 1 - (ngy ? 1 : 0);
            const int lz = s.ck + 1 - (ngz ? 1 : 0);
            rx = lx - oA.x;
            ry = ly - oA.y;
            rz = lz - oA.z;
            const bool hx = ngx != flx, hy = ngy != fly, hz = ngz != flz;
            X0 = lx + (hx ? 1 : 0); X1 = lx + (hx ? 0 : 1);
            Y0 = ly + (hy ? 1 : 0); Y1 = ly + (hy ? 0 : 1);
            Z0 = lz + (hz ? 1 : 0); Z1 = lz + (hz ? 0 : 1);
        }
        if (CBET && CBET_LANES(live)) {
            double ds = 0.0;
            if (gk || CBET >= 2) ds = sqrt_speed(__builtin_fma(s.vz, s.vz, __builtin_fma(s.vy, s.vy, s.vx * s.vx))) * a.dt;
            double u_eff = s.uray;
            if (gk) {
                const double x = gain_exponent<IDX64>(a, gk, X0, X1, Y0, Y1, Z0, Z1, Fx0, Fx1, Fy0, Fy1, Fz0, Fz1, sXh, sYh, ds);
                const double phi = gain_phi(x, (CBET_BALLOT(!(fabs(x) < kPhiSmallBelow)) & live) == 0ull);
                const double dg = s.uray * (x * phi);
                u_eff = s.uray * phi;
                gained += dg;
                s.uray = s.uray + dg;
            }
            if (CBET == 2) q0 = u_eff * ds;
            if (CBET == 4) {
                q0 = u_eff * ds;
                q1 = u_eff * (s.vx * a.dt);
                q2 = u_eff * (s.vy * a.dt);
                q3 = u_eff * (s.vz * a.dt);
                const int hi = s.ci + 1, hj = s.cj + 1, hk = s.ck + 1;
                own_slot = T::slot_d(hi & T::XM, hj & T::YM, hk & T::ZM) + NSLOT;
                own_node = __mul24(hi, sXh) + __mul24(hj, sYh) + hk;
            }
        }
        const unsigned long long memA = live & ~hbm;
        unsigned long long out_core = memA & ~(CBET_BALLOT((unsigned)rx <= (unsigned)T::SX) & CBET_BALLOT((unsigned)ry <= (unsigned)T::SY) &
                                               CBET_BALLOT((unsigned)rz <= (unsigned)T::SZ));
        if (CBET_RARE(b_active != 0)) {
            asm volatile("");
            if constexpr (STATS) wc.slabs_bsteps += 1u;
            const int abx = oA.x - oB.x, aby = oA.y - oB.y, abz = oA.z - oB.z;
            out_core |= hbm & ~(CBET_BALLOT((unsigned)(rx + abx) <= (unsigned)TB::SX) &
                                CBET_BALLOT((unsigned)(ry + aby) <= (unsigned)TB::SY) &
                                CBET_BALLOT((unsigned)(rz + abz) <= (unsigned)TB::SZ));
            tile_off = CBET_LANES(hbm) ? T::N : 0;
        }
        out_core |= miss_m;
        if (CBET_RARE(out_core != 0ull)) {
            wc.dg.arm_begin();
            const bool alive = CBET_LANES(live);
            int lx = rx + oA.x, ly = ry + oA.y, lz = rz + oA.z;
            asm volatile("" : "+v"(lx), "+v"(ly), "+v"(lz));
            Origin nA = oA, nB = oB;
            unsigned long long n_hbm = hbm, n_miss = 0ull;
            int n_bact = b_active, n_near, n_toff = tile_off;
            follow_box<T, NC>(a, tileA, nA, memA, lx, ly, lz, lane, edep, sXh, sYh, wc, NSLOT, a.comp_stride);
            const unsigned long long lost_mask =
                memA & ~(CBET_BALLOT((unsigned)(lx - nA.x) <= (unsigned)T::SX) & CBET_BALLOT((unsigned)(ly - nA.y) <= (unsigned)T::SY) &
                         CBET_BALLOT((unsigned)(lz - nA.z) <= (unsigned)T::SZ));
            if (CBET_USUAL(lost_mask == 0ull && n_bact == 0)) {
                n_near = box_near_axes<T>(nA, nx, ny, nz);
            } else {
                bool homeB = CBET_LANES(hbm);
                const bool inA = alive && holds<T>(nA, lx, ly, lz);
                const bool lost = alive && !homeB && !inA;
                if (n_bact != 0) {
                    follow_box<TB, 1>(a, tileB, nB, hbm, lx, ly, lz, lane, edep, sXh, sYh, wc, 0, 0);
                } else if (lost_mask != 0ull) {
                    const int src = __ffsll((long long)lost_mask) - 1;
                    const int sx = __builtin_amdgcn_readlane(lx, src), sy = __builtin_amdgcn_readlane(ly, src),
                              sz = __builtin_amdgcn_readlane(lz, src);
                    nB.x = sx - (TB::WX / 2 - 1);
                    nB.y = sy - (TB::WY / 2 - 1);
                    nB.z = sz - TB::SZ / 2;
                    n_bact = 1;
                }
                const bool inB = alive && holds<TB>(nB, lx, ly, lz);
                homeB = homeB || (lost && inB);
                if (alive && homeB && !inB && inA) homeB = false;
                n_hbm = CBET_BALLOT(alive && homeB);
                if (n_hbm == 0ull) {
                    __builtin_amdgcn_wave_barrier();
                    flush_box<TB, 1>(a, tileB, nB, lane, edep, sXh, sYh, wc, 0, 0);
                    n_bact = 0;
                }
                __builtin_amdgcn_wave_barrier();
                const bool useB = alive && homeB && inB;
                n_toff = useB ? T::N : 0;
                n_miss = live & ~CBET_BALLOT(useB || (alive && !homeB && inA));
                if constexpr (STATS) {
                    if (n_miss != 0ull) wc.steps_miss += 1u;
                    if (ACC && CBET_LANES(n_miss)) ++wc.n_miss;
                }
                n_near = n_miss != 0ull ? 7 : (box_near_axes<T>(nA, nx, ny, nz) | (n_bact == 0 ? 0 : box_near_axes<TB>(nB, nx, ny, nz)));
            }
            commit(oA.x, nA.x); commit(oA.y, nA.y); commit(oA.z, nA.z);
            commit(oB.x, nB.x); commit(oB.y, nB.y); commit(oB.z, nB.z);
            commit(hbm, n_hbm); commit(miss_m, n_miss);
            commit(b_active, n_bact); commit(near, n_near);
            commit_v(tile_off, n_toff);
            wc.pend = __builtin_amdgcn_readfirstlane(wc.pend);
            wc.dg.arm_end();
        } else if (CBET_RARE(near != 0)) {
            commit(near, box_near_axes<T>(oA, nx, ny, nz) | (b_active == 0 ? 0 : box_near_axes<TB>(oB, nx, ny, nz)));
        }
        step_tail(tt);
    }
    tot_steps += __popcll(live) * a.nt;

    if constexpr (PIPE) accumulate();
    if constexpr (ACC) flush_sums(live & ~miss_m, live & miss_m);
    else deposit_step(live & ~miss_m, live & miss_m);
    __syncthreads();
    flush_box<T, NC>(a, tileA, oA, lane, edep, sXh, sYh, wc, NSLOT, a.comp_stride);
    if (b_active != 0) flush_box<TB, 1>(a, tileB, oB, lane, edep, sXh, sYh, wc, 0, 0);

    if (CBET && a.beam_gain) {
        double t = gained;
#pragma unroll
        for (int off = 32; off > 0; off >>= 1) t += __shfl_xor(t, off, kWave);
        if (lane == 0 && t != 0.0) atomicAdd(&a.beam_gain[beam], t);
    }
    if (wc.dg.report(a, lane, tot_steps, tot_rays, wc.steps_miss >> 16)) return;
    if constexpr (STATS) {
        const int tot_at = wave_sum(wc.n_atomics), tot_miss = wave_sum(wc.n_miss);
        if (lane == 0) {
            atomicAdd(&a.counters[kCntGlobalAtomics], (unsigned long long)tot_at);
            atomicAdd(&a.counters[kCntEvictions], (unsigned long long)tot_miss);
            atomicAdd(&a.counters[kCntWaveSteps], (unsigned long long)(wc.steps_miss >> 16));
            atomicAdd(&a.counters[kCntWaveStepsMiss], (unsigned long long)(wc.steps_miss & 0xFFFFu));
            atomicAdd(&a.counters[kCntWaveStepsWide], (unsigned long long)(wc.slabs_bsteps & 0xFFFFu));
            atomicAdd(&a.counters[kCntSlabsRetired], (unsigned long long)(wc.slabs_bsteps >> 16));
        }
    }
    if (lane == 0) {
        atomicAdd(&a.counters[kCntSteps], (unsigned long long)tot_steps);
        atomicAdd(&a.counters[kCntRays], (unsigned long long)tot_rays);
    }
}

}

hipError_t launch_trace_window(const TraceArgs &a, bool force_idx64, hipStream_t stream)
{
    const long waves = a.item_count;
    if (waves <= 0) return hipSuccess;
    const dim3 grid((unsigned)waves), block(kWave);
    const unsigned long long grid_bytes = 8ull * (unsigned long long)a.sXh * (unsigned long long)(a.nx + 2);
    const bool generic = force_idx64 || (a.gain && 8ull * (unsigned long long)a.hsize >= (1ull << 32)) || a.absorption != 1 ||
                         grid_bytes >= (1ull << 32) ||
                         sizeof(StepRecord) * (unsigned long long)a.nx * a.ny * a.nz > (1ull << 32);
    auto go = [&](auto wz, auto cbet) {
        constexpr int WZ = decltype(wz)::value, CB = decltype(cbet)::value;
        if (a.stats) {
            if (generic) hipLaunchKernelGGL((k_trace_window<WZ, true, CB, true>), grid, block, 0, stream, a);
            else hipLaunchKernelGGL((k_trace_window<WZ, false, CB, true>), grid, block, 0, stream, a);
        } else {
            if (generic) hipLaunchKernelGGL((k_trace_window<WZ, true, CB, false>), grid, block, 0, stream, a);
            else hipLaunchKernelGGL((k_trace_window<WZ, false, CB, false>), grid, block, 0, stream, a);
        }
    };
    using std::integral_constant;
    if (a.quantity == 1) go(integral_constant<int, 8>{}, integral_constant<int, 4>{});
    else if (a.quantity == 2) go(integral_constant<int, 16>{}, integral_constant<int, 2>{});
    else if (a.gain || a.beam_gain) go(integral_constant<int, 16>{}, integral_constant<int, 1>{});
    else go(integral_constant<int, 16>{}, integral_constant<int, 0>{});
    return hipGetLastError();
}

}
```

Before: 174.8 billion.

## Precompute per-ray launch records and per-beam launch tables; overlap launch with record gather

```diff
diff --git a/cbet_raytracing_3d_amd/build.py b/cbet_raytracing_3d_amd/build.py
--- a/cbet_raytracing_3d_amd/build.py
+++ b/cbet_raytracing_3d_amd/build.py
@@ -12,7 +12,7 @@
            "cbet_target.hip", "cbet_mesh.hip", "cbet_mesh_deposit.hip", "cbet_params.cpp", "cbet_context.cpp", "cbet_tables_abi.cpp", "cbet_trace_abi.cpp", "cbet_gain_abi.cpp",
            "cbet_host.cpp", "cbet_output.cpp", "cbet_sph_host.cpp", "cbet_target_host.cpp", "cbet_mesh_host.cpp", "cbet_mesh_deposit_host.cpp",
            "cbet_exchange_host.cpp"]
-HEADERS = [os.path.join(CSRC, "cbet_device.h"), os.path.join(CSRC, "cbet_host_internal.h"), os.path.join(CSRC, "cbet_relocate.h"), os.path.join(CSRC, "cbet_trace_common.h"), os.path.join(CSRC, "cbet_trace_diag.h"), os.path.join(CSRC, "cbet_hd.h"), os.path.join(CSRC, "cbet_node_model.h"), os.path.join(CSRC, "cbet_node_kernel.h"), os.path.join(CSRC, "cbet_target_model.h"), os.path.join(CSRC, "cbet_mesh_model.h"), os.path.join(CSRC, "cbet_state_model.h"), os.path.join(CSRC, "cbet_mesh_deposit_model.h"), os.path.join(CSRC, "cbet_gain_model.h"), os.path.join(ROOT, "include", "cbet_mi355x.h"),
+HEADERS = [os.path.join(CSRC, "cbet_device.h"), os.path.join(CSRC, "cbet_host_internal.h"), os.path.join(CSRC, "cbet_relocate.h"), os.path.join(CSRC, "cbet_trace_common.h"), os.path.join(CSRC, "cbet_trace_diag.h"), os.path.join(CSRC, "cbet_hd.h"), os.path.join(CSRC, "cbet_launch_model.h"), os.path.join(CSRC, "cbet_node_model.h"), os.path.join(CSRC, "cbet_node_kernel.h"), os.path.join(CSRC, "cbet_target_model.h"), os.path.join(CSRC, "cbet_mesh_model.h"), os.path.join(CSRC, "cbet_state_model.h"), os.path.join(CSRC, "cbet_mesh_deposit_model.h"), os.path.join(CSRC, "cbet_gain_model.h"), os.path.join(ROOT, "include", "cbet_mi355x.h"),
            os.path.join(ROOT, "include", "cbet_omega_beams.h")]
 
 FLAGS = ["-O3", "-std=c++17", "--offload-arch=gfx950", "-ffp-contract=off", "-fPIC", "-shared",
diff --git a/cbet_raytracing_3d_amd/csrc/cbet_context.cpp b/cbet_raytracing_3d_amd/csrc/cbet_context.cpp
--- a/cbet_raytracing_3d_amd/csrc/cbet_context.cpp
+++ b/cbet_raytracing_3d_amd/csrc/cbet_context.cpp
@@ -52,6 +52,34 @@
     return CBET_OK;
 }
 
+static hipError_t upload_launch_list(cbet_context *ctx, const int *list, size_t n, const char **what)
+{
+    std::vector<LaunchRecord> rec(n);
+    for (size_t i = 0; i < n; ++i)
+        rec[i] = launch_record(list[i], ctx->xlaunch_host.data(), ctx->ylaunch_host.data(), ctx->p.rays_per_zone, ctx->d.zones_spanned);
+    const size_t m = std::max<size_t>(1, n);
+    int *live = nullptr;
+    LaunchRecord *drec = nullptr;
+    double *power = nullptr;
+    hipError_t e;
+    auto undo = [&](hipError_t err, const char *w) {
+        (void)hipFree(live); (void)hipFree(drec); (void)hipFree(power);
+        *what = w;
+        return err;
+    };
+    if ((e = hipMalloc((void **)&live, m * sizeof(int))) != hipSuccess) return undo(e, "hipMalloc(live)");
+    if ((e = hipMalloc((void **)&drec, m * sizeof(LaunchRecord))) != hipSuccess) return undo(e, "hipMalloc(launch records)");
+    if ((e = hipMalloc((void **)&power, m * sizeof(double))) != hipSuccess) return undo(e, "hipMalloc(launch power)");
+    if (n && (e = hipMemcpy(live, list, n * sizeof(int), hipMemcpyHostToDevice)) != hipSuccess) return undo(e, "hipMemcpy(live)");
+    if (n && (e = hipMemcpy(drec, rec.data(), n * sizeof(LaunchRecord), hipMemcpyHostToDevice)) != hipSuccess) return undo(e, "hipMemcpy(launch records)");
+    (void)hipFree(ctx->live); (void)hipFree(ctx->launch_rec); (void)hipFree(ctx->launch_power);
+    ctx->live = live;
+    ctx->launch_rec = drec;
+    ctx->launch_power = power;
+    ctx->nlive = (int)n;
+    return hipSuccess;
+}
+
 extern "C" {
 
 int cbet_safeGPUAlloc(void **dst, size_t size, int gpu)
@@ -97,10 +125,11 @@
     (void)hipFree(ctx->ne3d);
     (void)hipFree(ctx->kap3d);
     (void)hipFree(ctx->steprec);
-    (void)hipFree(ctx->xlaunch);
-    (void)hipFree(ctx->ylaunch);
     (void)hipFree(ctx->bounds);
     (void)hipFree(ctx->live);
+    (void)hipFree(ctx->launch_rec);
+    (void)hipFree(ctx->launch_power);
+    (void)hipFree(ctx->beam_launch);
     (void)hipFree(ctx->counters);
     (void)hipFree(ctx->flow_own);
     (void)hipFree(ctx->state_own);
@@ -130,13 +159,9 @@
     std::sort(want.begin(), want.end());
     std::sort(got.begin(), got.end());
     if (want != got) return fail(CBET_EINVAL, "the launch list must hold exactly the context's live rays, each once (%zu given, %zu expected)", got.size(), want.size());
-    int *fresh = nullptr;
-    CBET_HIP(hipMalloc((void **)&fresh, (size_t)n * sizeof(int)));
-    hipError_t e = hipMemcpy(fresh, list, (size_t)n * sizeof(int), hipMemcpyHostToDevice);
-    if (e != hipSuccess) { (void)hipFree(fresh); return fail_hip(CBET_EHIP, "hipMemcpy(launch list): %s", hipGetErrorString(e)); }
-    (void)hipFree(ctx->live);
-    ctx->live = fresh;
-    ctx->nlive = (int)n;
+    const char *what = "";
+    hipError_t e = upload_launch_list(ctx, list, (size_t)n, &what);
+    if (e != hipSuccess) return fail_hip(e == hipErrorOutOfMemory ? CBET_ENOMEM : CBET_EHIP, "%s (launch list): %s", what, hipGetErrorString(e));
     return CBET_OK;
 }
 
@@ -156,7 +181,8 @@
     ctx->gpu = gpu;
     ctx->p = *p;
     ctx->d = d;
-    ctx->nlive = (int)live.size();
+    ctx->xlaunch_host = xl;
+    ctx->ylaunch_host = yl;
     const size_t nodes = (size_t)p->nx * p->ny * p->nz;
     auto bail = [&](hipError_t err, const char *what) {
         cbet_context_destroy(ctx);
@@ -165,21 +191,18 @@
     if ((e = hipMalloc((void **)&ctx->ne3d, nodes * sizeof(double))) != hipSuccess) return bail(e, "hipMalloc(ne3d)");
     if ((e = hipMalloc((void **)&ctx->kap3d, nodes * sizeof(double))) != hipSuccess) return bail(e, "hipMalloc(kappa3d)");
     if ((e = hipMalloc((void **)&ctx->steprec, nodes * sizeof(StepRecord))) != hipSuccess) return bail(e, "hipMalloc(step records)");
-    if ((e = hipMalloc((void **)&ctx->xlaunch, xl.size() * sizeof(double))) != hipSuccess) return bail(e, "hipMalloc(xlaunch)");
-    if ((e = hipMalloc((void **)&ctx->ylaunch, yl.size() * sizeof(double))) != hipSuccess) return bail(e, "hipMalloc(ylaunch)");
     if ((e = hipMalloc((void **)&ctx->bounds, 6 * sizeof(double))) != hipSuccess) return bail(e, "hipMalloc(bounds)");
     {
         double hb[6];
         host_exit_planes(p, d, hb);
         if ((e = hipMemcpy(ctx->bounds, hb, sizeof hb, hipMemcpyHostToDevice)) != hipSuccess) return bail(e, "hipMemcpy(bounds)");
     }
-    if ((e = hipMalloc((void **)&ctx->live, std::max<size_t>(1, live.size()) * sizeof(int))) != hipSuccess) return bail(e, "hipMalloc(live)");
+    {
+        const char *what = "";
+        if ((e = upload_launch_list(ctx, live.data(), live.size(), &what)) != hipSuccess) return bail(e, what);
+    }
+    if ((e = hipMalloc((void **)&ctx->beam_launch, (size_t)p->nbeams * kBeamLaunchDoubles * sizeof(double))) != hipSuccess) return bail(e, "hipMalloc(beam launch table)");
     if ((e = hipMalloc((void **)&ctx->counters, kCntSlots * sizeof(unsigned long long))) != hipSuccess) return bail(e, "hipMalloc(counters)");
-    if ((e = hipMemcpy(ctx->xlaunch, xl.data(), xl.size() * sizeof(double), hipMemcpyHostToDevice)) != hipSuccess) return bail(e, "hipMemcpy(xlaunch)");
-    if ((e = hipMemcpy(ctx->ylaunch, yl.data(), yl.size() * sizeof(double), hipMemcpyHostToDevice)) != hipSuccess) return bail(e, "hipMemcpy(ylaunch)");
-    if (!live.empty() &&
-        (e = hipMemcpy(ctx->live, live.data(), live.size() * sizeof(int), hipMemcpyHostToDevice)) != hipSuccess)
-        return bail(e, "hipMemcpy(live)");
     if ((e = hipMemset(ctx->counters, 0, kCntSlots * sizeof(unsigned long long))) != hipSuccess) return bail(e, "hipMemset(counters)");
     if ((e = target_upload_factors()) != hipSuccess) return bail(e, "hipMemcpyToSymbol(target factors)");
     *out = ctx;
diff --git a/cbet_raytracing_3d_amd/csrc/cbet_device.h b/cbet_raytracing_3d_amd/csrc/cbet_device.h
--- a/cbet_raytracing_3d_amd/csrc/cbet_device.h
+++ b/cbet_raytracing_3d_amd/csrc/cbet_device.h
@@ -3,6 +3,7 @@
 
 #include <hip/hip_runtime_api.h>
 
+#include "cbet_launch_model.h"
 #include "cbet_mi355x.h"
 
 namespace cbet {
@@ -14,9 +15,9 @@
 constexpr double kLambda = 1.053e-4 / 3.0;
 constexpr double kSigma = 0.0375;
 constexpr double kIntensity = 1.0e14;
-constexpr double kFocal = 0.1;
+constexpr double kFocal = kLaunchFocal;
 constexpr double kBeamMin = -450.0e-4;
-constexpr double kBeamMax = 450.0e-4;
+constexpr double kBeamMax = kLaunchBeamMax;
 
 constexpr unsigned kEmptyTag = 0xFFFFFFFFu;
 constexpr int kWave = 64;
@@ -61,18 +62,17 @@
     double tol_x, tol_y, tol_z;
     double xconst, yconst, zconst;
     int nt, absorption;
-    int rpz, zones, nrays_x;
     double z_launch;
     double uray_mult, omega, ncrit;
-    const double *xlaunch, *ylaunch;
-    const int *live;
+    const LaunchRecord *launch_rec;
+    const double *launch_power;
+    const double *beam_launch;
     int nlive;
     int beam_lo, nbeams_local, bundles_per_beam;
     long total_bundles;
     long first_item, item_count;
     const double *ne3d, *kap3d;
     const StepRecord *steprec;
-    const double *beam_norm, *bbeam_norm, *pow_r, *phase_r;
     double *edep;
     int sYh, sXh;
     long grid_stride;
@@ -112,6 +112,17 @@
     const double *shift;
 };
 
+struct LaunchTableArgs {
+    const LaunchRecord *rec;
+    int nlive;
+    const double *pow_r, *phase_r;
+    double *power;
+    const double *beam_norm, *bbeam_norm;
+    int beam_lo, nbeams_local;
+    double *beam_launch;
+};
+
+hipError_t launch_launch_tables(const LaunchTableArgs &a, hipStream_t stream);
 hipError_t launch_tabulate(const TabulateArgs &a, hipStream_t stream);
 hipError_t launch_step_table(const StepTableArgs &a, hipStream_t stream);
 hipError_t launch_plasma_records(const PlasmaRecordsArgs &a, hipStream_t stream);
diff --git a/cbet_raytracing_3d_amd/csrc/cbet_host_internal.h b/cbet_raytracing_3d_amd/csrc/cbet_host_internal.h
--- a/cbet_raytracing_3d_amd/csrc/cbet_host_internal.h
+++ b/cbet_raytracing_3d_amd/csrc/cbet_host_internal.h
@@ -18,10 +18,13 @@
     unsigned long long rec_builds = 0;
     const double *rec_ne3d = nullptr, *rec_kap3d = nullptr;
     double rec_const[3] = {0, 0, 0};
-    double *xlaunch = nullptr, *ylaunch = nullptr;
     double *bounds = nullptr;
     int *live = nullptr;
     int nlive = 0;
+    std::vector<double> xlaunch_host, ylaunch_host;
+    cbet::LaunchRecord *launch_rec = nullptr;
+    double *launch_power = nullptr;
+    double *beam_launch = nullptr;
     unsigned long long *counters = nullptr;
     double *flow_own = nullptr;
     const double *flow = nullptr;
@@ -77,6 +80,8 @@
 int check_geometry(const cbet_context *ctx, const cbet_params *p);
 int entry_checks(const cbet_context *ctx, const cbet_params *p);
 int default_context(const cbet_params *p, cbet_context **out);
+LaunchTableArgs launch_table_args(const cbet_context *ctx, const double *pow_r, const double *phase_r, const double *beam_norm,
+                                  const double *bbeam_norm, int beam_lo, int beam_hi);
 
 template <class Args>
 void grid_dims(Args &a, const cbet_params *p)
diff --git a/cbet_raytracing_3d_amd/csrc/cbet_kernels.hip b/cbet_raytracing_3d_amd/csrc/cbet_kernels.hip
--- a/cbet_raytracing_3d_amd/csrc/cbet_kernels.hip
+++ b/cbet_raytracing_3d_amd/csrc/cbet_kernels.hip
@@ -339,10 +339,35 @@
     }
 }
 
+__global__ void __launch_bounds__(256) k_launch_tables(const LaunchTableArgs a)
+{
+    const long t = (long)blockIdx.x * blockDim.x + threadIdx.x;
+    if (t < a.nlive) a.power[t] = interp_table(a.pow_r, a.phase_r, a.rec[t].ref, CBET_NPHASE);
+    if (t < a.nbeams_local) {
+        const int beam = a.beam_lo + (int)t;
+        double *out = a.beam_launch + (long)beam * kBeamLaunchDoubles;
+        beam_direction(a.beam_norm + 3 * beam, out + kBlDir);
+        out[3] = 0.0;
+        if (a.bbeam_norm) {
+            for (int q = 0; q < 4; ++q) out[kBlTrig + q] = a.bbeam_norm[4 * beam + q];
+        } else {
+            beam_trig(a.beam_norm + 3 * beam, out + kBlTrig);
+        }
+    }
+}
+
 #ifdef CBET_DEBUG_BOUNDS
 __device__ unsigned long long g_audit_violations;
 #endif
 
+}
+
+hipError_t launch_launch_tables(const LaunchTableArgs &a, hipStream_t stream)
+{
+    const long threads = a.nlive > a.nbeams_local ? a.nlive : a.nbeams_local;
+    if (threads <= 0) return hipSuccess;
+    hipLaunchKernelGGL(k_launch_tables, dim3((unsigned)((threads + 255) / 256)), dim3(256), 0, stream, a);
+    return hipGetLastError();
 }
 
 hipError_t launch_tabulate(const TabulateArgs &a, hipStream_t stream)
diff --git a/cbet_raytracing_3d_amd/csrc/cbet_launch_model.h b/cbet_raytracing_3d_amd/csrc/cbet_launch_model.h
--- /dev/null
+++ b/cbet_raytracing_3d_amd/csrc/cbet_launch_model.h
@@ -0,0 +1,86 @@
+#ifndef CBET_LAUNCH_MODEL_H_
+#define CBET_LAUNCH_MODEL_H_
+
+#include <math.h>
+
+#include "cbet_hd.h"
+
+namespace cbet {
+
+constexpr double kLaunchBeamMax = 450.0e-4;
+constexpr double kLaunchFocal = 0.1;
+
+enum LaunchState { kLaunchRay = 0, kLaunchHole = 1, kLaunchCulled = 2 };
+struct alignas(16) LaunchRecord {
+    double x0, y0, ref;
+    int state, pad;
+};
+static_assert(sizeof(LaunchRecord) == 32, "two 16-byte loads per lane");
+
+CBET_HD LaunchRecord launch_record(int pre_raynum, const double *xlaunch, const double *ylaunch, int rpz, int zones)
+{
+    LaunchRecord r = {0.0, 0.0, 0.0, kLaunchHole, 0};
+    if (pre_raynum < 0) return r;
+    const int rpz2 = rpz * rpz;
+    const int tile = pre_raynum / rpz2, within = pre_raynum % rpz2;
+    const int ry = tile / zones * rpz + within / rpz;
+    const int rx = tile % zones * rpz + within % rpz;
+    const double x0 = xlaunch[rx];
+    const double y0 = ylaunch[ry];
+    r.x0 = x0;
+    r.y0 = y0;
+    r.ref = sqrt(x0 * x0 + y0 * y0);
+    r.state = !(r.ref <= kLaunchBeamMax) ? kLaunchCulled : kLaunchRay;
+    return r;
+}
+
+CBET_HD double interp_table(const double *y, const double *x, const double xp, int n)
+{
+    unsigned lo, hi, mid;
+    if (x[0] <= x[n - 1]) {
+        if (xp <= x[0]) return y[0];
+        if (xp >= x[n - 1]) return y[n - 1];
+        lo = 0;
+        hi = n - 1;
+        mid = (lo + hi) >> 1;
+        while (lo < hi - 1) {
+            if (x[mid] >= xp) hi = mid; else lo = mid;
+            mid = (lo + hi) >> 1;
+        }
+    } else {
+        if (xp >= x[0]) return y[0];
+        if (xp <= x[n - 1]) return y[n - 1];
+        lo = 0;
+        hi = n - 1;
+        mid = (lo + hi) >> 1;
+        while (lo < hi - 1) {
+            if (x[mid] <= xp) lo = mid; else hi = mid;
+            mid = (lo + hi) >> 1;
+        }
+    }
+    return y[mid] + (y[mid + 1] - y[mid]) / (x[mid + 1] - x[mid]) * (xp - x[mid]);
+}
+
+constexpr int kBeamLaunchDoubles = 8, kBlDir = 0, kBlTrig = 4;
+
+CBET_HD void beam_direction(const double *bn, double *dir)
+{
+    const double vx = -1 * bn[0], vy = -1 * bn[1], vz = -1 * bn[2];
+    const double knorm = sqrt(vx * vx + vy * vy + vz * vz);
+    dir[0] = vx / knorm;
+    dir[1] = vy / knorm;
+    dir[2] = vz / knorm;
+}
+
+CBET_HD void beam_trig(const double *bn, double *trig)
+{
+    const double theta1 = acos(bn[2]);
+    const double theta2 = atan2(bn[1] * kLaunchFocal, kLaunchFocal * bn[0]);
+    trig[0] = cos(theta1);
+    trig[1] = sin(theta1);
+    trig[2] = cos(theta2);
+    trig[3] = sin(theta2);
+}
+
+}
+#endif
diff --git a/cbet_raytracing_3d_amd/csrc/cbet_trace_abi.cpp b/cbet_raytracing_3d_amd/csrc/cbet_trace_abi.cpp
--- a/cbet_raytracing_3d_amd/csrc/cbet_trace_abi.cpp
+++ b/cbet_raytracing_3d_amd/csrc/cbet_trace_abi.cpp
@@ -1,6 +1,18 @@
 #include "cbet_host_internal.h"
 
 using namespace cbet;
+
+LaunchTableArgs cbet::launch_table_args(const cbet_context *ctx, const double *pow_r, const double *phase_r, const double *beam_norm,
+                                        const double *bbeam_norm, int beam_lo, int beam_hi)
+{
+    LaunchTableArgs t{};
+    t.rec = ctx->launch_rec; t.nlive = ctx->nlive;
+    t.pow_r = pow_r; t.phase_r = phase_r; t.power = ctx->launch_power;
+    t.beam_norm = beam_norm; t.bbeam_norm = bbeam_norm;
+    t.beam_lo = beam_lo; t.nbeams_local = beam_hi - beam_lo;
+    t.beam_launch = ctx->beam_launch;
+    return t;
+}
 
 int cbet::trace_impl(int b, unsigned nindices, const double *ne3d, const double *kappa3d, double *edep,
                      const double *bbeam_norm, const double *beam_norm, const double *pow_r, const double *phase_r,
@@ -47,11 +59,10 @@
     a.tol_x = 0.5001 * d.dx; a.tol_y = 0.5001 * d.dy; a.tol_z = 0.5001 * d.dz;
     a.xconst = xconst; a.yconst = yconst; a.zconst = zconst;
     a.nt = d.nt; a.absorption = p->absorption;
-    a.rpz = p->rays_per_zone; a.zones = d.zones_spanned; a.nrays_x = d.nrays_x;
     a.z_launch = kFocal - d.dz / 2;
     a.uray_mult = d.uray_mult; a.omega = d.omega; a.ncrit = d.ncrit;
-    a.xlaunch = ctx->xlaunch; a.ylaunch = ctx->ylaunch;
-    a.live = ctx->live; a.nlive = ctx->nlive;
+    a.launch_rec = ctx->launch_rec; a.launch_power = ctx->launch_power; a.beam_launch = ctx->beam_launch;
+    a.nlive = ctx->nlive;
     a.beam_lo = beam_lo; a.nbeams_local = beam_hi - beam_lo;
     a.bundles_per_beam = (ctx->nlive + kWave - 1) / kWave;
     a.total_bundles = (long)a.nbeams_local * a.bundles_per_beam;
@@ -62,7 +73,6 @@
     }
     a.ne3d = ne3d ? ne3d : ctx->ne3d;
     a.kap3d = kappa3d ? kappa3d : ctx->kap3d;
-    a.beam_norm = beam_norm; a.bbeam_norm = bbeam_norm; a.pow_r = pow_r; a.phase_r = phase_r;
     a.edep = edep;
     a.sYh = p->edep_zpitch > 0 ? p->edep_zpitch : p->nz + 2;
     a.sXh = (p->ny + 2) * a.sYh;
@@ -85,6 +95,7 @@
         if (int rc = step_records(ctx, p, ne3d, kappa3d, xconst, yconst, zconst, stream, false)) return rc;
         a.steprec = ctx->steprec;
     }
+    CBET_HIP(launch_launch_tables(launch_table_args(ctx, pow_r, phase_r, beam_norm, bbeam_norm, beam_lo, beam_hi), (hipStream_t)stream));
     CBET_HIP(launch_trace(a, hooks.exits ? kTraceExits : variant, p->force_wide_index != 0, (hipStream_t)stream));
     return CBET_OK;
 }
diff --git a/cbet_raytracing_3d_amd/csrc/cbet_trace_common.h b/cbet_raytracing_3d_amd/csrc/cbet_trace_common.h
--- a/cbet_raytracing_3d_amd/csrc/cbet_trace_common.h
+++ b/cbet_raytracing_3d_amd/csrc/cbet_trace_common.h
@@ -7,33 +7,6 @@
 #include "cbet_relocate.h"
 
 namespace cbet {
-
-__device__ __forceinline__ double interp_table(const double *y, const double *x, const double xp, int n)
-{
-    unsigned lo, hi, mid;
-    if (x[0] <= x[n - 1]) {
-        if (xp <= x[0]) return y[0];
-        if (xp >= x[n - 1]) return y[n - 1];
-        lo = 0;
-        hi = n - 1;
-        mid = (lo + hi) >> 1;
-        while (lo < hi - 1) {
-            if (x[mid] >= xp) hi = mid; else lo = mid;
-            mid = (lo + hi) >> 1;
-        }
-    } else {
-        if (xp >= x[0]) return y[0];
-        if (xp <= x[n - 1]) return y[n - 1];
-        lo = 0;
-        hi = n - 1;
-        mid = (lo + hi) >> 1;
-        while (lo < hi - 1) {
-            if (x[mid] <= xp) lo = mid; else hi = mid;
-            mid = (lo + hi) >> 1;
-        }
-    }
-    return y[mid] + (y[mid + 1] - y[mid]) / (x[mid + 1] - x[mid]) * (xp - x[mid]);
-}
 
 struct Ray {
     double px, py, pz, vx, vy, vz, uray, ustop;
@@ -56,33 +29,16 @@
     return found;
 }
 
-__device__ __forceinline__ bool launch_ray(const TraceArgs &a, int beam, int pre_raynum, Ray &s)
-{
-    const int rpz = a.rpz, rpz2 = rpz * rpz;
-    const int tile = pre_raynum / rpz2, within = pre_raynum % rpz2;
-    const int ry = tile / a.zones * rpz + within / rpz;
-    const int rx = tile % a.zones * rpz + within % rpz;
-    double x0 = a.xlaunch[rx];
-    double y0 = a.ylaunch[ry];
-    const double ref = sqrt(x0 * x0 + y0 * y0);
+__device__ __forceinline__ bool launch_point(const TraceArgs &a, int beam, int patch, int lane, Ray &s, int &li)
+{
+    li = patch * kWave + lane;
+    if (!(li < a.nlive)) return false;
+    const LaunchRecord r = a.launch_rec[li];
+    if (r.state == kLaunchHole) return false;
+    double x0 = r.x0, y0 = r.y0;
     double z0 = a.z_launch;
-
-    const double bnx = a.beam_norm[beam * 3 + 0], bny = a.beam_norm[beam * 3 + 1],
-                 bnz = a.beam_norm[beam * 3 + 2];
-    double c1, s1, c2, s2;
-    if (a.bbeam_norm) {
-        c1 = a.bbeam_norm[4 * beam + 0];
-        s1 = a.bbeam_norm[4 * beam + 1];
-        c2 = a.bbeam_norm[4 * beam + 2];
-        s2 = a.bbeam_norm[4 * beam + 3];
-    } else {
-        const double theta1 = acos(bnz);
-        const double theta2 = atan2(bny * kFocal, kFocal * bnx);
-        c1 = cos(theta1);
-        s1 = sin(theta1);
-        c2 = cos(theta2);
-        s2 = sin(theta2);
-    }
+    const double *bl = a.beam_launch + beam * kBeamLaunchDoubles + kBlTrig;
+    const double c1 = bl[0], s1 = bl[1], c2 = bl[2], s2 = bl[3];
     const double keep = x0;
     x0 = x0 * c1 + z0 * s1;
     z0 = z0 * c1 - keep * s1;
@@ -93,29 +49,34 @@
     s.px = x0;
     s.py = y0;
     s.pz = z0;
-    s.uray = a.uray_mult * interp_table(a.pow_r, a.phase_r, ref, CBET_NPHASE);
+    s.uray = a.uray_mult * a.launch_power[li];
     s.ustop = 0.05 * s.uray;
-    if (!(ref <= kBeamMax)) return false;
+    if (r.state != kLaunchRay) return false;
 
     s.ci = first_node_within(s.px, a.xmin, a.dx, a.tol_x, a.nx);
     s.cj = first_node_within(s.py, a.ymin, a.dy, a.tol_y, a.ny);
     s.ck = first_node_within(s.pz, a.zmin, a.dz, a.tol_z, a.nz);
-
-    const double ne0 = a.ne3d[((long)s.ci * a.ny + s.cj) * a.nz + s.ck];
+    return true;
+}
+
+__device__ __forceinline__ double launch_density(const TraceArgs &a, const Ray &s)
+{
+    return a.ne3d[((long)s.ci * a.ny + s.cj) * a.nz + s.ck];
+}
+__device__ __forceinline__ void launch_velocity(const TraceArgs &a, int beam, double ne0, Ray &s)
+{
     const double w = sqrt((a.omega * a.omega - ne0 * 1e6 * (kEc * kEc) / ((double)kMe * kE0)) / (kC * kC));
-    double vx = -1 * bnx, vy = -1 * bny, vz = -1 * bnz;
-    const double knorm = sqrt(vx * vx + vy * vy + vz * vz);
-    s.vx = (kC * kC) * ((vx / knorm) * w) / a.omega;
-    s.vy = (kC * kC) * ((vy / knorm) * w) / a.omega;
-    s.vz = (kC * kC) * ((vz / knorm) * w) / a.omega;
-    return true;
+    const double *dir = a.beam_launch + beam * kBeamLaunchDoubles + kBlDir;
+    s.vx = (kC * kC) * (dir[0] * w) / a.omega;
+    s.vy = (kC * kC) * (dir[1] * w) / a.omega;
+    s.vz = (kC * kC) * (dir[2] * w) / a.omega;
 }
 
 __device__ __forceinline__ bool launch_lane(const TraceArgs &a, int beam, int patch, int lane, Ray &s, int &li)
 {
-    li = patch * kWave + lane;
-    const int pre_raynum = li < a.nlive ? a.live[li] : -1;
-    return pre_raynum >= 0 && launch_ray(a, beam, pre_raynum, s);
+    if (!launch_point(a, beam, patch, lane, s, li)) return false;
+    launch_velocity(a, beam, launch_density(a, s), s);
+    return true;
 }
 
 template <class T = int> __device__ __forceinline__ void face_pair(int c, int n, T &m, T &p, T stride = 1)
diff --git a/cbet_raytracing_3d_amd/csrc/cbet_trace_diag.h b/cbet_raytracing_3d_amd/csrc/cbet_trace_diag.h
--- a/cbet_raytracing_3d_amd/csrc/cbet_trace_diag.h
+++ b/cbet_raytracing_3d_amd/csrc/cbet_trace_diag.h
@@ -24,7 +24,7 @@
 struct WaveDiag {
     typedef unsigned long long u64;
     static constexpr bool kCountsWaveSteps = (0 CBET_IF_CLOCKS(+1) CBET_IF_FACES(+1) CBET_IF_CHAIN(+1)) != 0;
-    CBET_IF_CLOCKS(u64 wait = 0, arm = 0, n_arm = 0, ret = 0, n_ret = 0, t_start, t_wait, t_arm, t_ret;)
+    CBET_IF_CLOCKS(u64 wait = 0, arm = 0, n_arm = 0, ret = 0, n_ret = 0, t_entry, t_start, t_wait, t_arm, t_ret;)
     CBET_IF_FACES(unsigned near_steps = 0, near_axes = 0, arm_steps = 0;)
     CBET_IF_CHAIN(u64 chain = 0, t_chain = 0;)
 
@@ -37,6 +37,7 @@
         return t1 - t0;
     }
 
+    __device__ __forceinline__ void entry() { CBET_IF_CLOCKS(stamp_wait(t_entry);) }
     __device__ __forceinline__ void begin() { CBET_IF_CLOCKS(stamp_wait(t_start);) }
     __device__ __forceinline__ void step_begin(int near)
     {
@@ -69,9 +70,13 @@
             put(kCntGlobalAtomics, wait);
             put(kCntEvictions, arm);
             put(kCntWaveStepsWide, n_arm);
-            put(kCntSlabsRetired, t_end - t_start);
+            put(kCntSlabsRetired, t_end - t_entry);
             put(kCntRays, ret);
+#if CBET_DIAG_CLOCKS + 0 >= 2
+            put(kCntWaveStepsMiss, t_start - t_entry);
+#else
             put(kCntWaveStepsMiss, n_ret);
+#endif
 #elif defined(CBET_DIAG_CHAIN)
             put(kCntRays, (u64)tot_rays);
             put(kCntGlobalAtomics, chain);
diff --git a/cbet_raytracing_3d_amd/csrc/cbet_trace_window.hip b/cbet_raytracing_3d_amd/csrc/cbet_trace_window.hip
--- a/cbet_raytracing_3d_amd/csrc/cbet_trace_window.hip
+++ b/cbet_raytracing_3d_amd/csrc/cbet_trace_window.hip
@@ -459,6 +459,8 @@
     constexpr int NLDS = NSLOT + (NC - 1) * T::DT;
     __shared__ double s_val[NLDS];
     const int lane = threadIdx.x;
+    WaveCounters wc;
+    wc.dg.entry();
 
     int beam, patch;
     if (!work_item(a, blockIdx.x, beam, patch)) return;
@@ -467,7 +469,7 @@
 
     Ray s = {};
     int li;
-    const bool launched = launch_lane(a, beam, patch, lane, s, li);
+    const bool launched = launch_point(a, beam, patch, lane, s, li);
     unsigned long long live = __ballot(launched);
     if (live == 0ull) return;
     const int tot_rays = __popcll(live);
@@ -477,23 +479,6 @@
     unsigned cell = launched ? (unsigned)((s.ci * ny + s.cj) * nz + s.ck) : 0u;
     double fcx = (double)s.ci, fcy = (double)s.cj, fcz = (double)s.ck;
     int tot_steps = 0;
-    WaveCounters wc;
-
-    double *const tileA = s_val, *const tileB = s_val + T::N;
-    Origin oA{0, 0, 0}, oB{0, 0, 0};
-    unsigned long long hbm = 0ull;
-    int b_active = 0;
-    {
-        const int src = ((live >> 27) & 1ull) ? 27 : (__ffsll((long long)live) - 1);
-        for (int z = lane; z < NLDS; z += kWave) s_val[z] = 0.0;
-        oA.x = __builtin_amdgcn_readlane(s.ci, src) + 1 - T::WX / 2;
-        oA.y = __builtin_amdgcn_readlane(s.cj, src) + 1 - T::WY / 2;
-        oA.z = __builtin_amdgcn_readlane(s.ck, src) + 1 - 4;
-        if (T::BRICK) oA.z &= ~7;
-        __syncthreads();
-    }
-    int near = 7;
-    wc.dg.begin();
 
     dbl2 rec_kxy, rec_kzk;
     const StepRecord *rec_base = a.steprec;
@@ -508,13 +493,31 @@
         record_issue<IDX64>(rec_base, c, rec_kxy, rec_kzk);
         wc.pend = 0;
     };
+    gather_record();
+    if (launched) launch_velocity(a, beam, launch_density(a, s), s);
+
+    double *const tileA = s_val, *const tileB = s_val + T::N;
+    Origin oA{0, 0, 0}, oB{0, 0, 0};
+    unsigned long long hbm = 0ull;
+    int b_active = 0;
+    {
+        const int src = ((live >> 27) & 1ull) ? 27 : (__ffsll((long long)live) - 1);
+        for (int z = lane; z < NLDS; z += kWave) s_val[z] = 0.0;
+        oA.x = __builtin_amdgcn_readlane(s.ci, src) + 1 - T::WX / 2;
+        oA.y = __builtin_amdgcn_readlane(s.cj, src) + 1 - T::WY / 2;
+        oA.z = __builtin_amdgcn_readlane(s.ck, src) + 1 - 4;
+        if (T::BRICK) oA.z &= ~7;
+        __syncthreads();
+    }
+    int near = 7;
+    wc.dg.begin();
+
     auto await_record = [&]() {
         wc.dg.wait_begin();
         if (CBET == 0 && !kAudited) record_wait(rec_kxy, rec_kzk, wc.pend);
         else record_wait_all(rec_kxy, rec_kzk);
         wc.dg.wait_end();
     };
-    gather_record();
     await_record();
     const double *const gk = CBET && a.gain ? a.gain + (long)(beam - a.grid_beam0) * a.hsize : nullptr;
     double gained = 0.0;
```

Result: no change. 175.7 billion (median of 3 runs) (+0.5%).
